# cp2k/dbcsr

Hardware: AMD Instinct MI355X
Metric: block-sparse multiply GFLOP/s (fp64) (higher is better)
Workload: dtype f64; 1 GPU; config2_32768_23x23_fill10_fp64; M=32768, c_nblks=2030625, nproducts=29207882, k_passes=1, parallelism=1 GPU

## Files before the change

### dbcsr_amd/csrc/mm_aux.h

```cpp
#ifndef DBCSR_AMD_MM_AUX_H
#define DBCSR_AMD_MM_AUX_H
#include "mm_epilogue.h"

namespace dbcsr_amd {

template <typename T>
__global__ void __launch_bounds__(256) checksum_blocks(const int* __restrict__ row_p, const int* __restrict__ col_i,
                                                       const int64_t* __restrict__ blk_p, const T* __restrict__ data,
                                                       const int* __restrict__ rs, const int* __restrict__ cs,
                                                       const int64_t* __restrict__ roff, const int64_t* __restrict__ coff, int nbr,
                                                       double* __restrict__ row_sums) {
  const int lane = threadIdx.x & 63;
  const int row = (blockIdx.x * blockDim.x + threadIdx.x) >> 6;
  if (row >= nbr) return;
  const int m = rs[row];
  double s2 = 0.0, sp = 0.0;
  for (int b = row_p[row]; b < row_p[row + 1]; ++b) {
    const int c = col_i[b];
    const int n = cs[c];
    const T* d = data + blk_p[b];
    for (int e = lane; e < m * n; e += 64) {
      const double x = (double)d[e];
      const int r = e % m, cc = e / m;
      s2 += x * x;
      sp += x * log(fabs((double)(roff[row] + r + 1) * (double)(coff[c] + cc + 1)));
    }
  }
  s2 = wave_sum(s2);
  sp = wave_sum(sp);
  if (lane == 0) {
    row_sums[2 * row] = s2;
    row_sums[2 * row + 1] = sp;
  }
}

__global__ void __launch_bounds__(256) checksum_final(const double* __restrict__ row_sums, int nbr, double* __restrict__ out2) {
  __shared__ double r2[256], rp[256];
  double s2 = 0.0, sp = 0.0;
  for (int i = threadIdx.x; i < nbr; i += 256) {
    s2 += row_sums[2 * i];
    sp += row_sums[2 * i + 1];
  }
  r2[threadIdx.x] = s2;
  rp[threadIdx.x] = sp;
  __syncthreads();
  for (int off = 128; off > 0; off >>= 1) {
    if ((int)threadIdx.x < off) {
      r2[threadIdx.x] += r2[threadIdx.x + off];
      rp[threadIdx.x] += rp[threadIdx.x + off];
    }
    __syncthreads();
  }
  if (threadIdx.x == 0) {
    out2[0] = r2[0];
    out2[1] = rp[0];
  }
}

__device__ __forceinline__ uint64_t larnv_block_seed(int irow, int nrow, int icol, int ival) {
  long long ivm = ((long long)ival) % 65536;
  if (ivm < 0) ivm += 65536;
  long long map = (((long long)irow - 1 + (long long)icol * (long long)nrow) * (1 + ivm)) * 2 + 1;
  const uint64_t s4 = (uint64_t)(map % 4096);
  map /= 4096;
  const uint64_t s3 = (uint64_t)((map ^ 3541) % 4096);
  map /= 4096;
  const uint64_t s2 = (uint64_t)((map ^ 1153) % 4096);
  map /= 4096;
  const uint64_t s1 = (uint64_t)((map ^ 2029) % 4096);
  return (s1 << 36) | (s2 << 24) | (s3 << 12) | s4;
}

__device__ __forceinline__ uint64_t pow48(uint64_t base, uint64_t e) {
  const uint64_t mask = (1ull << 48) - 1;
  uint64_t r = 1;
  base &= mask;
  while (e) {
    if (e & 1) r = (r * base) & mask;
    base = (base * base) & mask;
    e >>= 1;
  }
  return r;
}

__global__ void __launch_bounds__(256) fill_random_f64(const int* __restrict__ row_p, const int* __restrict__ col_i,
// ... 322 lines not shown
struct Window {
  int r0, r1, c0, c1;
};

__global__ void __launch_bounds__(256) crop_flags(const int* __restrict__ row_p, const int* __restrict__ col_i, const int* __restrict__ rs,
                                                  const int* __restrict__ cs, const int64_t* __restrict__ roff,
                                                  const int64_t* __restrict__ coff, int nbr, Window w, int* __restrict__ keep,
                                                  int* __restrict__ blk_nze, int* __restrict__ row_keep) {
  const int lane = threadIdx.x & 63;
  const int row = (blockIdx.x * blockDim.x + threadIdx.x) >> 6;
  if (row >= nbr) return;
  const int m = rs[row];
  const bool row_in = roff[row] + m - 1 >= w.r0 && roff[row] <= w.r1;
  int cnt = 0;
  for (int b = row_p[row] + lane; b < row_p[row + 1]; b += 64) {
    const int c = col_i[b], n = cs[c];
    const int k = (row_in && coff[c] + n - 1 >= w.c0 && coff[c] <= w.c1) ? 1 : 0;
    keep[b] = k;
    blk_nze[b] = k ? m * n : 0;
    cnt += k;
  }
  cnt = wave_sum(cnt);
  if (lane == 0) row_keep[row] = cnt;
}

template <typename T>
__global__ void __launch_bounds__(256) crop_compact(const int* __restrict__ row_p, const int* __restrict__ col_i,
                                                    const int64_t* __restrict__ blk_p, const T* __restrict__ data,
                                                    const int* __restrict__ rs, const int* __restrict__ cs,
                                                    const int64_t* __restrict__ roff, const int64_t* __restrict__ coff, int nbr, Window w,
                                                    const int* __restrict__ keep, const int64_t* __restrict__ newidx,
                                                    const int64_t* __restrict__ newoff, int* __restrict__ d_col_i,
                                                    int64_t* __restrict__ d_blk_p, T* __restrict__ d_data) {
  const int lane = threadIdx.x & 63;
  const int row = (blockIdx.x * blockDim.x + threadIdx.x) >> 6;
  if (row >= nbr) return;
  const int m = rs[row];
  const int64_t r_base = roff[row];
  for (int b = row_p[row]; b < row_p[row + 1]; ++b) {
    if (!keep[b]) continue;
    const int64_t t = newidx[b], off = newoff[b];
    const int c = col_i[b];
    if (lane == 0) {
      d_col_i[t] = c;
      d_blk_p[t] = off;
    }
    const int ne = m * cs[c];
    const int64_t c_base = coff[c];
    const T* src = data + blk_p[b];
    T* dst = d_data + off;
    for (int e = lane; e < ne; e += 64) {
      const int64_t gr = r_base + e % m, gc = c_base + e / m;
      dst[e] = (gr >= w.r0 && gr <= w.r1 && gc >= w.c0 && gc <= w.c1) ? src[e] : T(0);
    }
  }
}

template <typename T>
__global__ void __launch_bounds__(256) scale_window(const int* __restrict__ row_p, const int* __restrict__ col_i,
                                                    const int64_t* __restrict__ blk_p, T* __restrict__ data, const int* __restrict__ rs,
                                                    const int* __restrict__ cs, const int64_t* __restrict__ roff,
                                                    const int64_t* __restrict__ coff, int nbr, Window w, T beta) {
  const int lane = threadIdx.x & 63;
  const int row = (blockIdx.x * blockDim.x + threadIdx.x) >> 6;
  if (row >= nbr) return;
  const int m = rs[row];
  const int64_t r_base = roff[row];
  if (r_base + m - 1 < w.r0 || r_base > w.r1) return;
  for (int b = row_p[row]; b < row_p[row + 1]; ++b) {
    const int c = col_i[b], n = cs[c];
    const int64_t c_base = coff[c];
    if (c_base + n - 1 < w.c0 || c_base > w.c1) continue;
    T* blk = data + blk_p[b];
    for (int e = lane; e < m * n; e += 64) {
      const int64_t gr = r_base + e % m, gc = c_base + e / m;
      if (gr >= w.r0 && gr <= w.r1 && gc >= w.c0 && gc <= w.c1) blk[e] *= beta;
    }
  }
}



constexpr int kStatSlots = 8192;
__global__ void __launch_bounds__(256) build_work(const int* __restrict__ order, int64_t npos, const Desc* __restrict__ descs, int64_t nblk,
                                                  const Entry* __restrict__ entries, Work* __restrict__ work) {
  const int64_t pos = (int64_t)blockIdx.x * blockDim.x + threadIdx.x;
  if (pos >= npos) return;
  const int cb = order[pos];
  Work w;
  w.c_off = 0, w.cin_off = -1, w.prod_start = 0, w.prod_cnt = -1, w.m = 0, w.n = 0, w.a_lo = 0, w.b_lo = 0, w.w = 0, w.cb = cb;
  if (cb >= 0 && cb < nblk) {
    const Desc d = descs[cb];
    w.c_off = d.c_off, w.cin_off = d.cin_off, w.prod_start = d.prod_start, w.prod_cnt = d.prod_cnt, w.m = d.m, w.n = d.n;
    if (d.prod_cnt > 0) {
      const Entry e = entries[d.prod_start];
      w.a_lo = e.a_lo, w.b_lo = e.b_lo, w.w = e.w;
    }
  }
  work[pos] = w;
}

__global__ void __launch_bounds__(256) mnk_histogram(const Desc* __restrict__ descs, int64_t nblk, const Entry* __restrict__ entries,
                                                     unsigned long long* __restrict__ keys, unsigned long long* __restrict__ counts,
                                                     int* __restrict__ overflow) {
  const int64_t cb = (int64_t)blockIdx.x * blockDim.x + threadIdx.x;
  if (cb >= nblk) return;
  const Desc d = descs[cb];
  const Entry* e = entries + d.prod_start;
  unsigned long long run_key = 0, run_cnt = 0;
  auto flush = [&]() {
    if (!run_cnt) return;
    unsigned h = (unsigned)((run_key * 0x9E3779B97F4A7C15ull) >> 40) & (kStatSlots - 1);
    for (int probe = 0; probe < kStatSlots; ++probe) {
      const unsigned long long prev = atomicCAS(&keys[h], 0ull, run_key);
      if (prev == 0ull || prev == run_key) {
        atomicAdd(&counts[h], run_cnt);
        return;
      }
      h = (h + 1) & (kStatSlots - 1);
    }
    *overflow = 1;
  };
  for (int p = 0; p < d.prod_cnt; ++p) {
    const unsigned long long key = (unsigned long long)(uint16_t)d.m | ((unsigned long long)(uint16_t)d.n << 16) |
                                   ((unsigned long long)(unsigned)e[p].ks() << 32) | (1ull << 63);
    if (key != run_key) {
      flush();
      run_key = key;
      run_cnt = 0;
    }
    ++run_cnt;
  }
  flush();
}

}
#endif
```

### dbcsr_amd/csrc/mm_choose.h

```cpp
#ifndef DBCSR_AMD_MM_CHOOSE_H
#define DBCSR_AMD_MM_CHOOSE_H

#include <algorithm>
#include <cstddef>
#include <cstdint>
#include <cstdio>

namespace dbcsr_amd {

#define DBCSR_AMD_HOT_SIZES(X) \
  X(9) X(10) X(11) X(12) X(13) X(14) X(15) X(16) X(17) X(18) X(19) X(20) X(21) X(22) X(23) X(24) X(25) X(26) X(27) X(28) X(29) X(30) X(31) X(32)
#define DBCSR_AMD_DMA_SIZES(X) X(13) X(16) X(23) X(32)
#define DBCSR_AMD_F32_DIRECT_SIZES(X) X(16) X(24) X(32)
#define DBCSR_AMD_MID_SHAPES(X)                                                                             \
  X(6, 8) X(6, 9) X(6, 10) X(6, 11) X(6, 12)                                                                \
  X(7, 9) X(7, 10) X(7, 11) X(7, 12)                                                                        \
  X(8, 6) X(8, 8) X(8, 9) X(8, 10) X(8, 11) X(8, 12)                                                        \
  X(9, 6) X(9, 7) X(9, 8) X(9, 9) X(9, 10) X(9, 11) X(9, 12)                                                \
  X(10, 6) X(10, 7) X(10, 8) X(10, 9) X(10, 10) X(10, 11) X(10, 12)                                         \
  X(11, 6) X(11, 7) X(11, 8) X(11, 9) X(11, 10) X(11, 11) X(11, 12)                                         \
  X(12, 6) X(12, 7) X(12, 8) X(12, 9) X(12, 10) X(12, 11) X(12, 12)

#define DBCSR_AMD_IS_(S_) || s == S_
static inline bool hot_f64_has(int m, int n, int k) { const int s = m; return m == n && m == k && (false DBCSR_AMD_HOT_SIZES(DBCSR_AMD_IS_)); }
static inline bool dma_f64_has(int stages, int m, int n, int k) { const int s = m; return stages >= 2 && stages <= 4 && m == n && m == k && (false DBCSR_AMD_DMA_SIZES(DBCSR_AMD_IS_)); }
static inline bool f32_direct_has(int m, int n, int k) { const int s = m; return m == n && m == k && (false DBCSR_AMD_F32_DIRECT_SIZES(DBCSR_AMD_IS_)); }
#undef DBCSR_AMD_IS_
static inline bool big_f64_has(int tm, int tn) { return tm >= 2 && tm <= 5 && tn >= 2 && tn <= 5; }
static inline int big_tiles(int size) { return std::max(2, ((size + 7) / 8 + 1) / 2); }
static inline bool z64_has(int ma, int nc) { return ma >= 1 && ma <= 4 && nc >= 1 && nc <= 4; }
static inline int z64_tiles(int size) { return std::max(1, (std::min(size, 32) + 7) / 8); }
static inline constexpr int z64_slice_bytes(int ma, int nc) { return 8 * (8 * ma + 1) * 16 + 8 * nc * 9 * 16; }
static inline bool mid_f64_has(int rb, int cb) {
#define DBCSR_AMD_IS_(A_, B_) || (rb == A_ && cb == B_)
  return false DBCSR_AMD_MID_SHAPES(DBCSR_AMD_IS_);
#undef DBCSR_AMD_IS_
}

static inline bool mid_f64_serves(int m, int n, int class_mode) {
  const int rb = (m + 3) / 4, cb = (n + 3) / 4;
  const int lo = rb < cb ? rb : cb, hi = rb < cb ? cb : rb;
  if (lo < 6 || hi > 12 || hi < 8) return false;
  if (hi >= 11) return lo <= 10 || (m % 4 == 0 && n % 4 == 0);
  if (hi >= 9) return true;
  return class_mode > 0 && (lo == 8 || (lo == 6 && class_mode != 3));
}

struct SizeFacts {
  int max_m = 0, max_k = 0, max_n = 0, min_m = 0, min_k = 0, min_n = 0;
  int hot_m = 0, hot_n = 0, hot_k = 0;
  int hot_cnt_m = 0, hot_cnt_k = 0, hot_cnt_n = 0;
  int units_m = 0, units_cnt_m = 0, units_n = 0, units_cnt_n = 0;
  int nbr = 0, nbc = 0;
  int64_t c_nblks = 0, nproducts = 0, order_len = 0;
  bool cls_mode = false;
  int cls_m[3] = {0, 0, 0}, cls_n[3] = {0, 0, 0}, cls_k[3] = {0, 0, 0};
  bool retain = false;
  int canonical_c = 0;
  bool filter_active = false;
  bool fp64 = true;
  int skip_empty = 0;
  bool cplx = false;

  bool sizes_within(int s) const { return max_m <= s && max_k <= s && max_n <= s && min_m >= 1 && min_k >= 1 && min_n >= 1; }
  bool no_empty_dim() const { return min_m >= 1 && min_n >= 1 && min_k >= 1; }
  bool dominant_cube() const { return hot_m > 0 && hot_m == hot_n && hot_m == hot_k; }
  bool other_sizes() const { return hot_cnt_m < nbr || hot_cnt_n < nbc; }
};

struct Switches {
  int use_lds = 1;
  int use_pipe = -1, pipe_g = 8;
  int use_hot = 1;
  int use_tiny = 1;
  int use_small = 2;
  int small_group = 0;
  int use_mid = 1;
  int use_big = 1;
  int use_work = 1;
  int use_classes = 1;
  int wg_waves = 0;
  int f32_direct = 1;
};

struct LabSwitches {
#ifdef DBCSR_AMD_EXPERIMENTS
#define DBCSR_AMD_LAB_INT_ int
#else
#define DBCSR_AMD_LAB_INT_ static constexpr int
#endif
  DBCSR_AMD_LAB_INT_ dbg = 0;
  DBCSR_AMD_LAB_INT_ dma_stages = 0;
  DBCSR_AMD_LAB_INT_ hot_persistent = 0;
  DBCSR_AMD_LAB_INT_ hot_variant = 0;
  DBCSR_AMD_LAB_INT_ lds_pad = 0;
  DBCSR_AMD_LAB_INT_ class_g = 1;
  DBCSR_AMD_LAB_INT_ class_streams = 1;
  DBCSR_AMD_LAB_INT_ row_group = 0;
  DBCSR_AMD_LAB_INT_ f32_group = 0;
  DBCSR_AMD_LAB_INT_ f64_group = 0;
  DBCSR_AMD_LAB_INT_ use_tile = 0;
  DBCSR_AMD_LAB_INT_ use_band = 0;
#undef DBCSR_AMD_LAB_INT_
  bool variant_active() const { return (dbg & ~32) != 0 || dma_stages != 0 || hot_persistent != 0 || hot_variant != 0; }
};

static inline void top3_sizes(const int* hist, int* out) {
  int used[3] = {-1, -1, -1};
  for (int r = 0; r < 3; ++r) {
    int best = 0, bc = 0;
    for (int sz = 1; sz <= 32; ++sz)
      if (hist[sz] > bc && sz != used[0] && sz != used[1]) best = sz, bc = hist[sz];
    out[r] = best;
    used[r] = best ? best : -1;
  }
}
static inline void choose_classes(SizeFacts* f, const Switches& sw, const int* hist) {
  f->cls_mode = false;
  const bool hot_cube = f->hot_m >= 9 && f->dominant_cube();
  if (sw.use_classes > 0 && f->sizes_within(32) && !(f->max_m <= 4 && f->max_n <= 4) && (sw.use_classes > 1 || (!hot_cube && f->c_nblks >= 200000))) {
    top3_sizes(hist, f->cls_m);
    top3_sizes(hist + 33, f->cls_n);
    top3_sizes(hist + 66, f->cls_k);
    f->cls_mode = f->cls_m[0] > 0 && f->cls_n[0] > 0 && f->cls_k[0] > 0;
  }
}

enum class Family {
  f64_tiny, f64_small8, f64_mid, f64_classes, f64_hot, f64_pipe, f64_lds, f64_big, f64_generic, f32_classes, f32_direct, f32_hot, f32_lds, f32_generic,
  f64_group, f64_tile, f64_band, f64_dma, f64_persistent, f32_group,
  z64
};

struct NumericChoice {
  Family family = Family::f64_generic;
  char name[96] = "";
  int ww = 4;
  bool work = false, norms = false, leaves_norms = false;
  unsigned grid = 0;
  size_t lds_bytes = 0;
  int flags = 0;
  int lds_a = 0, lds_wave = 0, maxt = 0;
  int mid_rb = 0, mid_cb = 0, mid_class_mode = 0;
  int depth = 0, group = 0;
  bool slim = false;
  int variant = 0, group_R = 0;
};

static inline int choose_wg_waves(const SizeFacts& f, const Switches& sw) { return sw.wg_waves > 0 ? sw.wg_waves : (f.nproducts <= 32 * f.c_nblks ? 1 : 4); }

static inline void choose_mid_shape(const SizeFacts& f, const Switches& sw, const LabSwitches& lab, int* mid_rb, int* mid_cb) {
  *mid_rb = *mid_cb = 0;
  if (!(f.fp64 && sw.use_big && sw.use_mid && sw.use_lds && !f.cls_mode && f.max_m <= 48 && f.max_n <= 48 && f.no_empty_dim() && f.order_len > 0 &&
        !lab.variant_active() && sw.use_hot && sw.use_pipe != 1))
    return;
  const bool dom = f.hot_m > 0 && f.hot_n > 0, all_in = (f.min_m > 24 && f.min_n > 24) || f.max_m > 32 || f.max_n > 32;
  const int dm = dom ? f.hot_m : (all_in ? f.max_m : 0), dn = dom ? f.hot_n : (all_in ? f.max_n : 0);
  if (dm > 0 && dn > 0 && mid_f64_serves(dm, dn, 0)) *mid_rb = (dm + 3) / 4, *mid_cb = (dn + 3) / 4;
  if (*mid_rb && !dom) {
    const int mu = (std::max(f.max_m, f.max_n) + 3) / 4, fb = (mu > 10 || *mid_rb > 10 || *mid_cb > 10) ? 12 : 10;
    const bool single = *mid_rb == fb && *mid_cb == fb;
    const bool most = 10ll * f.units_cnt_m >= 8ll * f.nbr && 10ll * f.units_cnt_n >= 8ll * f.nbc && mid_f64_serves(4 * f.units_m, 4 * f.units_n, 0);
// ... 146 lines not shown
```

### dbcsr_amd/csrc/mm_engine.hip

```cpp
#include <hip/hip_runtime.h>

#include <cstdio>
#include <cstdlib>
#include <cstring>
#include <algorithm>
#include <new>
#include <vector>

#include "../../include/dbcsr_amd_mm.h"
#include "common.h"
#include "smm_core.h"
#include "mm_types.h"
#include "mm_complex.h"
#include "mm_jit.h"

#include "mm_workspace.h"
#include "mm_symbolic.h"
#include "mm_numeric_f64.h"
#include "mm_numeric_f64_big.h"
#include "mm_numeric_f64_small.h"
#include "mm_mid.h"
#include "mm_numeric_f32.h"
#include "mm_numeric_z64.h"
#include "mm_aux.h"
#include "mm_algebra.h"
#include "mm_elementwise.h"
#include "mm_blocklist.h"
#include "mm_multivec.h"
#include "mm_rank_update.h"
#include "mm_block_inverse.h"
#include "mm_block_scale.h"
#include "mm_dense.h"
#include "mm_submatrix.h"
#include "mm_csr.h"
#ifdef DBCSR_AMD_EXPERIMENTS
#include "mm_lab_api.h"
#include "mm_group.h"
#include "mm_group64.h"
#include "mm_dma.h"
#include "mm_tile_index.h"
#include "mm_band_index.h"
#endif
namespace dbcsr_amd {

#include "mm_engine_state.h"
#include "mm_engine_env.h"
#include "mm_engine_launch.h"
#include "mm_engine_plan.h"
#ifdef DBCSR_AMD_EXPERIMENTS
#include "mm_engine_lab.h"
#endif


static int build_product_lists(Engine* E, bool reuse, const dbcsr_amd_bcsr* a, const dbcsr_amd_bcsr* b, const dbcsr_amd_bcsr* c_in, dbcsr_amd_bcsr* c_out,
                               hipStream_t st) {
  const int nbr = E->facts.nbr, W = E->W, nbc = b->nblkcols, nJ = (nbc + 63) / 64;
  const int64_t nblk = E->facts.c_nblks;
  const uint32_t* cin_bm = E->have_cin ? E->cin_bm.p : nullptr;
  const int* cin_pre = E->have_cin ? E->cin_pre.p : nullptr;
  if (reuse) {
    ACC_CHECK(hipMemcpyAsync(c_out->col_i, E->plan_c_col_i.p, sizeof(int32_t) * (size_t)nblk, hipMemcpyDeviceToDevice, st));
    ACC_CHECK(hipMemcpyAsync(c_out->blk_p, E->plan_c_blk_p.p, sizeof(int64_t) * (size_t)nblk, hipMemcpyDeviceToDevice, st));
  } else if (E->rows_kernels) {
    if (E->tmp_i32.ensure((size_t)nblk + 1)) return -1;
    ACC_CHECK(hipMemsetAsync(E->tmp_i32.p, 0, sizeof(int) * (size_t)nblk, st));
    hipLaunchKernelGGL(fill_products_rows, grid_for((int64_t)nbr * 64), dim3(256), 0, st, a->row_p, a->col_i, a->blk_p, a->col_blk_size, b->row_p,
                       b->col_i, b->blk_p, E->c_bm.p, E->c_pre.p, c_out->row_p, E->prod_start.p, nbr, W, E->tmp_i32.p, E->entries.p, E->filter);
    hipLaunchKernelGGL(finish_descs_grid, grid_for((int64_t)nbr * nJ * 64), dim3(256), 0, st, c_in->row_p, c_in->blk_p, c_out->row_blk_size,
                       c_out->col_blk_size, cin_bm, cin_pre, E->c_bm.p, E->c_pre.p, c_out->row_p, E->c_blk_p_ws.p, E->prod_start.p,
                       E->prod_cnt.p, nbr, W, nJ, c_out->col_i, c_out->blk_p, E->descs.p);
  } else if (E->grid_kernels) {
    hipLaunchKernelGGL(fill_products_grid, grid_for((int64_t)nbr * nJ * 64), dim3(256), 0, st, a->row_p, a->col_i, a->blk_p, b->row_p,
                       b->blk_p, c_in->row_p, c_in->blk_p, a->row_blk_size, a->col_blk_size, b->col_blk_size, E->b_bm.p, E->b_pre.p,
                       cin_bm, cin_pre, E->c_bm.p, E->c_pre.p, c_out->row_p, E->prod_start.p, E->c_blk_p_ws.p, nbr, nbc, W, nJ, c_out->col_i,
                       c_out->blk_p, E->descs.p, E->entries.p, E->filter);
  } else {
    hipLaunchKernelGGL(fill_products, grid_for((int64_t)nbr * W), dim3(256), 0, st, a->row_p, a->col_i, a->blk_p, b->row_p, b->blk_p,
                       c_in->row_p, c_in->blk_p, a->row_blk_size, a->col_blk_size, b->col_blk_size, E->b_bm.p, E->b_pre.p,
                       cin_bm, cin_pre, E->c_bm.p, E->c_pre.p, c_out->row_p, E->prod_start.p, E->c_blk_p_ws.p, nbr, W, c_out->col_i, c_out->blk_p,
                       E->descs.p, E->entries.p);
  }
  return 0;
}

template <typename T>
static NumericArgs<T> numeric_args(Engine* E, hipStream_t st, const dbcsr_amd_bcsr* a, const dbcsr_amd_bcsr* b, const dbcsr_amd_bcsr* c_in,
                                   const dbcsr_amd_bcsr* c_out, T alpha, T beta, const Work* work, double* norms, bool reuse) {
  return NumericArgs<T>{st, E->descs.p, E->facts.c_nblks, E->entries.p, static_cast<const T*>(a->data), static_cast<const T*>(b->data),
                        static_cast<T*>(c_out->data), static_cast<const T*>(c_in->data), alpha, beta, E->facts.skip_empty, E->order.p, work, norms,
                        a, b, c_out, reuse};
}

static int launch_classes_f64(Engine* E, const NumericArgs<double>& p, const NumericChoice& c) {
  const SizeFacts& F = E->facts;
  int njit = 0, ngen = 0, nmid = 0, jit_mask = 0, nlaunch = 0;
  const int nside = E->lab.class_streams > 1 ? E->lab.class_streams - 1 : 0;
  if (nside) {
    if (!E->fork_ev) ACC_CHECK(hipEventCreateWithFlags(&E->fork_ev, hipEventDisableTiming));
    ACC_CHECK(hipEventRecord(E->fork_ev, p.st));
    for (int i = 0; i < nside; ++i) {
      if (!E->side_stream[i]) {
        ACC_CHECK(hipStreamCreateWithFlags(&E->side_stream[i], hipStreamNonBlocking));
        ACC_CHECK(hipEventCreateWithFlags(&E->join_ev[i], hipEventDisableTiming));
      }
      ACC_CHECK(hipStreamWaitEvent(E->side_stream[i], E->fork_ev, 0));
    }
  }
  for (int k = 0; k < kNumClasses; ++k) {
    if (E->cls_len[k] == 0) continue;
    NumericArgs<double> q = p.segment(E->cls_off[k]);
    const int slot = nlaunch++ % (nside + 1);
    if (slot) q.st = E->side_stream[slot - 1];
    const unsigned npos = (unsigned)(8 * E->cls_len[k]);
    const int cm = k < 9 ? F.cls_m[k / 3] : 0, cn = k < 9 ? F.cls_n[k % 3] : 0;
    ClassKernel ck;
    if (k < 9 && c.mid_class_mode && mid_f64_serves(cm, cn, c.mid_class_mode)) {
      if (!launch_mid_f64(q, (cm + 3) / 4, (cn + 3) / 4, false, npos, (std::max(cm, cn) + 3) / 4)) return -1;
      ++nmid;
      jit_mask |= 1 << k;
    } else if (k < 9 && cm > 0 && cn > 0 && jit_class_kernel(cm, cn, F.cls_k[0], F.cls_k[1], F.cls_k[2], E->lab.class_g, &ck) == 0) {
      long nblk_l = (long)q.nblk;
      void* args[] = {&q.descs, &nblk_l, &q.entries, &q.a, &q.b, &q.c_out, &q.c_in, &q.alpha, &q.beta, &q.skip_empty, &q.order, &q.work, &q.norms};
      const unsigned cw = E->lab.class_g == 1 ? (unsigned)c.ww : 4u;
      ACC_CHECK(hipModuleLaunchKernel(ck.fn, npos / cw / (unsigned)E->lab.class_g, 1, 1, 64 * cw, 1, 1, (unsigned)(cw * ck.wave_lds), q.st, args, nullptr));
      ++njit;
      jit_mask |= 1 << k;
    } else {
      launch_lds_f64(q, c, (unsigned)(8 * E->cls_len[k] / 4) * 4u / (unsigned)c.ww);
      ++ngen;
    }
  }
  for (int i = 0; i < nside; ++i) {
    ACC_CHECK(hipEventRecord(E->join_ev[i], E->side_stream[i]));
    ACC_CHECK(hipStreamWaitEvent(p.st, E->join_ev[i], 0));
  }
  if (p.norms) {
    ClassSet cs;
    for (int r = 0; r < 3; ++r) cs.m[r] = F.cls_m[r], cs.n[r] = F.cls_n[r];
    cs.jit_mask = jit_mask;
    hipLaunchKernelGGL(block_norms_unserved_classes, grid_for(p.nblk * 64), dim3(256), 0, p.st, p.descs, p.nblk, p.c_out, cs, p.norms);
  }
  char slab[24] = "";
  if (nmid > 0) snprintf(slab, sizeof slab, "%d slab + ", nmid);
  snprintf(E->last_kernel, sizeof E->last_kernel, "%s%d jit + %s%d generic launches; m {%d,%d,%d} n {%d,%d,%d} k {%d,%d,%d}]", c.name, njit, slab, ngen,
           F.cls_m[0], F.cls_m[1], F.cls_m[2], F.cls_n[0], F.cls_n[1], F.cls_n[2], F.cls_k[0], F.cls_k[1], F.cls_k[2]);
  return 0;
}

static int launch_f64(Engine* E, const NumericChoice& c, const NumericArgs<double>& p, const LabSwitches& lab) {
  const SizeFacts& F = E->facts;
  const int64_t npos = 8 * F.order_len;
  snprintf(E->last_kernel, sizeof E->last_kernel, "%s", c.name);
  if (p.norms && c.leaves_norms) E->norms_data = p.c_out, E->norms_nblks = p.nblk;
  switch (c.family) {
    case Family::f64_tiny:
      if (c.grid > 0) launch_tiny_f64(p, c, F.max_k <= 4);
      return 0;
    case Family::f64_small8:
      if (c.grid > 0) launch_small_f64(p, c, npos);
      return 0;
    case Family::f64_mid:
      return launch_mid_f64(p, c.mid_rb, c.mid_cb, F.min_m != F.max_m || F.min_n != F.max_n, c.grid, (std::max(F.max_m, F.max_n) + 3) / 4) ? 0 : -1;
    case Family::f64_classes: return launch_classes_f64(E, p, c);
    case Family::f64_hot: return launch_hot_f64(p, c, F.hot_m, F.hot_n, F.hot_k, c.flags, c.variant) ? 0 : -1;
    case Family::f64_pipe: launch_pipe_f64(p, c, npos); return 0;
    case Family::f64_lds: launch_lds_f64(p, c, c.grid); return 0;
    case Family::f64_big: return launch_big_f64(p, c, big_tiles(F.max_m), big_tiles(F.max_n)) ? 0 : -1;
    case Family::f64_generic:
      hipLaunchKernelGGL(mm_numeric_f64, dim3(c.grid), dim3(256), 0, p.st, p.descs, p.nblk, p.entries, p.a, p.b, p.c_out, p.c_in, p.alpha, p.beta, c.flags);
      return 0;
#ifdef DBCSR_AMD_EXPERIMENTS
    case Family::f64_group: case Family::f64_tile: case Family::f64_band: case Family::f64_dma: case Family::f64_persistent: return launch_lab_f64(E, c, p, lab);
#endif
    default: return -1;
  }
}

static int launch_f32(Engine* E, const NumericChoice& c, const NumericArgs<float>& p) {
  const SizeFacts& F = E->facts;
  snprintf(E->last_kernel, sizeof E->last_kernel, "%s", c.name);
  switch (c.family) {
    case Family::f32_classes:
      for (int k = 0; k < kNumClasses; ++k)
        if (E->cls_len[k] != 0) launch_lds_f32(p.segment(E->cls_off[k]), c, (unsigned)(8 * E->cls_len[k] / c.ww));
      return 0;
    case Family::f32_direct: return launch_hot_f32_direct(p, c, F.hot_m, F.hot_n, F.hot_k, c.flags, c.slim) ? 0 : -1;
    case Family::f32_hot: return launch_hot_f32(p, c, F.hot_m, F.hot_n, F.hot_k) ? 0 : -1;
    case Family::f32_lds: launch_lds_f32(p, c, c.grid); return 0;
    case Family::f32_generic:
      hipLaunchKernelGGL(mm_numeric_f32, dim3(c.grid), dim3(256), 0, p.st, p.descs, p.nblk, p.entries, p.a, p.b, p.c_out, p.c_in, p.alpha, p.beta, c.flags);
      return 0;
#ifdef DBCSR_AMD_EXPERIMENTS
    case Family::f32_group: {
      const int rc = run_group_f32(E, p, c.group_R);
      if (rc == 0 && F.other_sizes()) launch_hot_f32_direct(p, c, F.hot_m, F.hot_n, F.hot_k, c.flags | 2, false);
      if (rc != 1) return rc;
      LabSwitches lab = E->lab;
      lab.f32_group = 0;
      return launch_f32(E, choose_numeric(F, E->sw, lab), p);
    }
#endif
    default: return -1;
  }
}

static int launch_z64_family(Engine* E, const NumericChoice& c, const NumericArgs<z64>& p) {
  const SizeFacts& F = E->facts;
  snprintf(E->last_kernel, sizeof E->last_kernel, "%s", c.name);
  if (c.family != Family::z64) return -1;
  return launch_z64(p, c, z64_tiles(F.max_m), z64_tiles(F.max_n), 8 * F.order_len) ? 0 : -1;
}

static int numeric_phase(void* handle, libsmm_acc_data_t datatype, const double alpha[2], const dbcsr_amd_bcsr* a, const dbcsr_amd_bcsr* b,
                         const double beta[2], const dbcsr_amd_bcsr* c_in, dbcsr_amd_bcsr* c_out, void* stream);

}

using namespace dbcsr_amd;

extern "C" {

int dbcsr_amd_mm_create(void** handle) {
  if (!handle) return -1;
  Engine* E = new (std::nothrow) Engine();
  if (!E) return -1;
  hipError_t e = hipHostMalloc(reinterpret_cast<void**>(&E->host_scalars), 16 * sizeof(int64_t), hipHostMallocDefault);
  if (e != hipSuccess) {
    delete E;
    return check(e, "hipHostMalloc", __FILE__, __LINE__);
  }
  if (hipHostMalloc(reinterpret_cast<void**>(&E->cls_host_hist), 3 * 33 * sizeof(int), hipHostMallocDefault) != hipSuccess ||
      hipHostMalloc(reinterpret_cast<void**>(&E->cls_host_lens), (2 * kNumClasses + 1) * sizeof(int64_t), hipHostMallocDefault) != hipSuccess)
    return -1;
  if (hipHostMalloc(reinterpret_cast<void**>(&E->plan_host_flag), sizeof(int), hipHostMallocDefault) != hipSuccess) return -1;
  engine_read_env(E);
  for (int i = 0; i < 3; ++i) {
    e = hipEventCreate(&E->ev[i]);
    if (e != hipSuccess) return check(e, "hipEventCreate", __FILE__, __LINE__);
  }
  *handle = E;
  return 0;
}

int dbcsr_amd_mm_timing(void* handle, float* ms_fill, float* ms_numeric) {
  Engine* E = static_cast<Engine*>(handle);
  if (!E || !E->timed) return -1;
  ACC_CHECK(hipEventSynchronize(E->ev[2]));
  float f = 0.f, n = 0.f;
  ACC_CHECK(hipEventElapsedTime(&f, E->ev[0], E->ev[1]));
  ACC_CHECK(hipEventElapsedTime(&n, E->ev[1], E->ev[2]));
  if (ms_fill) *ms_fill = f;
  if (ms_numeric) *ms_numeric = n;
  return 0;
}

int dbcsr_amd_mm_destroy(void* handle) {
  if (!handle) return 0;
  Engine* E = static_cast<Engine*>(handle);
  if (E->host_scalars) (void)hipHostFree(E->host_scalars);
  if (E->plan_host_flag) (void)hipHostFree(E->plan_host_flag);
  if (E->cls_host_hist) (void)hipHostFree(E->cls_host_hist);
  if (E->cls_host_lens) (void)hipHostFree(E->cls_host_lens);
  for (int i = 0; i < 3; ++i)
    if (E->ev[i]) (void)hipEventDestroy(E->ev[i]);
  for (int i = 0; i < 3; ++i) {
    if (E->side_stream[i]) (void)hipStreamDestroy(E->side_stream[i]);
    if (E->join_ev[i]) (void)hipEventDestroy(E->join_ev[i]);
  }
  if (E->fork_ev) (void)hipEventDestroy(E->fork_ev);
  delete E;
  return 0;
}

int dbcsr_amd_mm_symbolic(void* handle, const dbcsr_amd_bcsr* a, const dbcsr_amd_bcsr* b, const dbcsr_amd_bcsr* c_in,
                          int retain_sparsity, int32_t* c_out_row_p, dbcsr_amd_mm_counts* counts, void* stream) {
  return dbcsr_amd_mm_symbolic_filtered(handle, dbcsr_type_real_8, 1.0, 0.0, a, b, c_in, retain_sparsity, c_out_row_p, counts, stream);
}

int dbcsr_amd_mm_symbolic_filtered(void* handle, libsmm_acc_data_t datatype, double alpha, double filter_eps, const dbcsr_amd_bcsr* a,
                                   const dbcsr_amd_bcsr* b, const dbcsr_amd_bcsr* c_in, int retain_sparsity, int32_t* c_out_row_p,
                                   dbcsr_amd_mm_counts* counts, void* stream) {
  Engine* E = static_cast<Engine*>(handle);
  if (!E || !a || !b || !c_in || !c_out_row_p || !counts) return -1;
  E->drop_pending = 0.0;
  engine_takes_work_areas(E);
  const bool filtering = filter_eps > 0.0;
  if (filtering && datatype != dbcsr_type_real_8 && datatype != dbcsr_type_real_4 && datatype != dbcsr_type_complex_8) return -10;
  if (a->nblkcols != b->nblkrows || a->nblkrows != c_in->nblkrows || b->nblkcols != c_in->nblkcols) {
    fprintf(stderr, "dbcsr_amd_mm_symbolic: incompatible block dimensions\n");
    return -2;
  }
  hipStream_t st = stream_of(stream);
  const int nbr = a->nblkrows, nbk = a->nblkcols, nbc = b->nblkcols;
  const int W = (nbc + 31) / 32;
  if (!filtering) {
    const int hit = plan_matches(E, a, b, c_in, retain_sparsity ? 1 : 0, st);
    if (hit < 0) return -1;
    if (hit) {
      long long off = 0;
      const void* ptr[12];
      long long n[12];
      plan_segments(a, b, c_in, ptr, n);
      for (int i = 0; i < 12; ++i) off += n[i];
      ACC_CHECK(hipMemcpyAsync(c_out_row_p, E->plan_words.p + off, sizeof(int32_t) * ((size_t)nbr + 1), hipMemcpyDeviceToDevice, st));
      *counts = E->plan_counts;
      E->norms_data = nullptr;
      E->filter = FilterArgs{nullptr, nullptr, 0.0f};
      E->valid = true;
      E->plan_hit = true;
      ++E->plan_hits;
      return 0;
    }
  }
  plan_invalidate(E);
  E->valid = false;
  E->facts.nbr = nbr;
  E->facts.nbc = nbc;
  E->W = W;
  E->facts.retain = retain_sparsity != 0;
  E->norms_data = nullptr;
  E->have_cin = c_in->nblks > 0;
  if (E->b_bm.ensure((size_t)nbk * W + 1) || E->b_pre.ensure((size_t)nbk * W + 1) || E->c_bm.ensure((size_t)nbr * W + 1) ||
      E->c_pre.ensure((size_t)nbr * W + 1) || E->row_nnz.ensure((size_t)nbr + 1) || E->dev_scalars.ensure(16))
    return -1;
  if (E->have_cin && (E->cin_bm.ensure((size_t)nbr * W + 1) || E->cin_pre.ensure((size_t)nbr * W + 1))) return -1;
  ACC_CHECK(hipMemsetAsync(E->dev_scalars.p, 0, 16 * sizeof(unsigned long long), st));
  {
    static const int init[6] = {0, -0x7fffffff, 0, -0x7fffffff, 0, -0x7fffffff};
    ACC_CHECK(hipMemcpyAsync(E->dev_scalars.p + 4, init, sizeof(init), hipMemcpyHostToDevice, st));
  }
  if (nbr == 0 || nbc == 0) {
    ACC_CHECK(hipMemsetAsync(c_out_row_p, 0, sizeof(int32_t) * ((size_t)nbr + 1), st));
    ACC_CHECK(hipStreamSynchronize(st));
    counts->c_nblks = counts->c_nze = counts->nproducts = counts->flop = 0;
    E->facts.c_nblks = 0;
    E->facts.nproducts = 0;
    E->grid_kernels = E->rows_kernels = false;
    E->facts.cls_mode = false;
    E->sym_bitmap = -1;
    E->sym_NP = E->sym_PW = E->sym_rowp_chunks = 0;
    E->valid = true;
    return 0;
  }
  ACC_CHECK(hipMemsetAsync(E->b_bm.p, 0, sizeof(uint32_t) * (size_t)nbk * W, st));
  if (nbk > 0) {
    hipLaunchKernelGGL(bitmap_from_index, grid_for((int64_t)nbk * 64), dim3(256), 0, st, b->row_p, b->col_i, nbk, W, E->b_bm.p);
    hipLaunchKernelGGL(row_prefix, grid_for((int64_t)nbk * 64), dim3(256), 0, st, E->b_bm.p, nbk, W, E->b_pre.p, (int*)nullptr);
  }
  if (E->have_cin) {
    ACC_CHECK(hipMemsetAsync(E->cin_bm.p, 0, sizeof(uint32_t) * (size_t)nbr * W, st));
    hipLaunchKernelGGL(bitmap_from_index, grid_for((int64_t)nbr * 64), dim3(256), 0, st, c_in->row_p, c_in->col_i, nbr, W,
                       E->cin_bm.p);
    hipLaunchKernelGGL(row_prefix, grid_for((int64_t)nbr * 64), dim3(256), 0, st, E->cin_bm.p, nbr, W, E->cin_pre.p, (int*)nullptr);
  }
  E->filter = FilterArgs{nullptr, nullptr, 0.0f};
  if (filtering) {
    if (E->a_norms.ensure((size_t)a->nblks + 1) || E->b_norms.ensure((size_t)b->nblks + 1)) return -1;
    const int sa = row_split(nbr, a->nblks), sb = row_split(nbk, b->nblks);
    if (datatype == dbcsr_type_real_8) {
      hipLaunchKernelGGL((bcsr_block_norms<double>), grid_for((int64_t)nbr * sa * 64), dim3(256), 0, st, a->row_p, a->col_i, a->blk_p,
                         static_cast<const double*>(a->data), a->row_blk_size, a->col_blk_size, nbr, sa, 1.0, E->a_norms.p, (double*)nullptr);
      hipLaunchKernelGGL((bcsr_block_norms<double>), grid_for((int64_t)nbk * sb * 64), dim3(256), 0, st, b->row_p, b->col_i, b->blk_p,
                         static_cast<const double*>(b->data), b->row_blk_size, b->col_blk_size, nbk, sb, alpha, E->b_norms.p, (double*)nullptr);
    } else if (datatype == dbcsr_type_complex_8) {
      hipLaunchKernelGGL((bcsr_block_norms<z64>), grid_for((int64_t)nbr * sa * 64), dim3(256), 0, st, a->row_p, a->col_i, a->blk_p,
                         static_cast<const z64*>(a->data), a->row_blk_size, a->col_blk_size, nbr, sa, 1.0, E->a_norms.p, (double*)nullptr);
      hipLaunchKernelGGL((bcsr_block_norms<z64>), grid_for((int64_t)nbk * sb * 64), dim3(256), 0, st, b->row_p, b->col_i, b->blk_p,
                         static_cast<const z64*>(b->data), b->row_blk_size, b->col_blk_size, nbk, sb, alpha, E->b_norms.p, (double*)nullptr);
    } else {
      hipLaunchKernelGGL((bcsr_block_norms<float>), grid_for((int64_t)nbr * sa * 64), dim3(256), 0, st, a->row_p, a->col_i, a->blk_p,
                         static_cast<const float*>(a->data), a->row_blk_size, a->col_blk_size, nbr, sa, 1.0, E->a_norms.p, (double*)nullptr);
      hipLaunchKernelGGL((bcsr_block_norms<float>), grid_for((int64_t)nbk * sb * 64), dim3(256), 0, st, b->row_p, b->col_i, b->blk_p,
                         static_cast<const float*>(b->data), b->row_blk_size, b->col_blk_size, nbk, sb, alpha, E->b_norms.p, (double*)nullptr);
    }
    E->filter = FilterArgs{E->a_norms.p, E->b_norms.p, (float)filter_eps};
  }
  SymbolicSizes sizes;
  sizes.nbr = nbr, sizes.nbk = nbk, sizes.nbc = nbc, sizes.a_nblks = a->nblks, sizes.b_nblks = b->nblks;
  sizes.filtering = filtering, sizes.retain = retain_sparsity != 0, sizes.forced = E->force_symbolic;
  SymbolicChoice sym = choose_symbolic_pattern(sizes);
  if (sym.bitmap_rows) {
    if (E->have_cin)
      ACC_CHECK(hipMemcpyAsync(E->c_bm.p, E->cin_bm.p, sizeof(uint32_t) * (size_t)nbr * W, hipMemcpyDeviceToDevice, st));
    else
      ACC_CHECK(hipMemsetAsync(E->c_bm.p, 0, sizeof(uint32_t) * (size_t)nbr * W, st));
    hipLaunchKernelGGL(c_bitmap_rows_filtered, grid_for((int64_t)nbr * 64), dim3(256), 0, st, a->row_p, a->col_i, b->row_p, b->col_i, nbr, W,
                       E->facts.canonical_c, E->filter, E->c_bm.p);
  } else if (filtering)
    hipLaunchKernelGGL(c_bitmap_filtered, grid_for((int64_t)nbr * ((nbc + 63) / 64) * 64), dim3(256), 0, st, a->row_p, a->col_i, b->row_p,
                       E->b_bm.p, E->b_pre.p, E->have_cin ? E->cin_bm.p : (const uint32_t*)nullptr, nbr, nbc, W, (nbc + 63) / 64,
                       retain_sparsity ? 1 : 0, E->facts.canonical_c, E->filter, E->c_bm.p);
  else
    hipLaunchKernelGGL(c_bitmap, grid_for((int64_t)nbr * W), dim3(256), 0, st, a->row_p, a->col_i, E->b_bm.p,
                       E->have_cin ? E->cin_bm.p : (const uint32_t*)nullptr, nbr, W, retain_sparsity ? 1 : 0, E->facts.canonical_c, E->c_bm.p);
  hipLaunchKernelGGL(row_prefix, grid_for((int64_t)nbr * 64), dim3(256), 0, st, E->c_bm.p, nbr, W, E->c_pre.p, E->row_nnz.p);
  int64_t* dsc = reinterpret_cast<int64_t*>(E->dev_scalars.p);
  if (exclusive_scan<int32_t>(E, E->row_nnz.p, nbr, c_out_row_p, dsc + 0, true, st)) return -1;
  if (E->sw.use_classes > 0 && E->cls_hist.ensure(3 * 33)) return -1;
  hipLaunchKernelGGL(block_size_stats, dim3(3), dim3(256), 0, st, a->row_blk_size, nbr, a->col_blk_size, nbk, b->col_blk_size, nbc,
                     reinterpret_cast<int*>(E->dev_scalars.p + 4), reinterpret_cast<int*>(E->dev_scalars.p + 8), reinterpret_cast<int*>(E->dev_scalars.p + 11),
                     E->sw.use_classes > 0 ? E->cls_hist.p : (int*)nullptr);
  if (E->sw.use_classes > 0) ACC_CHECK(hipMemcpyAsync(E->cls_host_hist, E->cls_hist.p, 3 * 33 * sizeof(int), hipMemcpyDeviceToHost, st));
  ACC_CHECK(hipMemcpyAsync(E->host_scalars, dsc, 13 * sizeof(int64_t), hipMemcpyDeviceToHost, st));
  ACC_CHECK(hipStreamSynchronize(st));
  const int64_t c_nblks = E->host_scalars[0];
  {
    const int* mx = reinterpret_cast<const int*>(E->host_scalars + 4);
    E->facts.max_m = mx[0]; E->facts.min_m = -mx[1];
    E->facts.max_k = mx[2]; E->facts.min_k = -mx[3];
    E->facts.max_n = mx[4]; E->facts.min_n = -mx[5];
    if (E->facts.max_k > 0xffff || E->facts.max_m > 0x7fff || E->facts.max_n > 0x7fff) {
      fprintf(stderr, "dbcsr_amd_mm_symbolic: block sizes above 32767 (m, n) / 65535 (k) are not supported (packed 16-bit extents)\n");
      return -1;
    }
    const int* md = reinterpret_cast<const int*>(E->host_scalars + 8);
    const bool dominant = 10ll * md[1] >= 9ll * nbr && 10ll * md[3] >= 9ll * nbk && 10ll * md[5] >= 9ll * nbc;
    E->facts.hot_m = dominant ? md[0] : 0;
    E->facts.hot_k = dominant ? md[2] : 0;
    E->facts.hot_n = dominant ? md[4] : 0;
    E->facts.hot_cnt_m = md[1], E->facts.hot_cnt_k = md[3], E->facts.hot_cnt_n = md[5];
    const int* um = reinterpret_cast<const int*>(E->host_scalars + 11);
    E->facts.units_m = um[0], E->facts.units_cnt_m = um[1], E->facts.units_n = um[2], E->facts.units_cnt_n = um[3];
  }
  E->facts.c_nblks = c_nblks;
  choose_classes(&E->facts, E->sw, E->cls_host_hist);
  double mean_k = E->facts.max_k, mean_n = E->facts.max_n;
  if (E->sw.use_classes > 0 && E->facts.max_k <= 32 && E->facts.max_n <= 32 && E->facts.min_k >= 1 && E->facts.min_n >= 1) {
    double sk = 0, ck = 0, sn = 0, cn = 0;
    for (int sz = 1; sz <= 32; ++sz) {
      sn += (double)sz * E->cls_host_hist[33 + sz];
      cn += E->cls_host_hist[33 + sz];
      sk += (double)sz * E->cls_host_hist[66 + sz];
      ck += E->cls_host_hist[66 + sz];
    }
    if (ck > 0 && cn > 0) mean_k = sk / ck, mean_n = sn / cn;
  }
  const int64_t b_bytes_est = (int64_t)((double)b->nblks * mean_k * mean_n * (double)sizeof(double));
  int NP = 1, PW = W;
  choose_panels(W, b_bytes_est, E->panel_bytes, &NP, &PW);
  const int R = (nbr + 7) / 8;
  int RG = E->lab.row_group > 0 ? E->lab.row_group : 1;
  RG = std::max(1, std::min(RG, R));
  const int NG = (R + RG - 1) / RG;
  const int nkeys = (E->facts.cls_mode ? kNumClasses : 1) * 8 * NP * (E->facts.cls_mode ? R : NG);
  if (E->order_cnt.ensure((size_t)nkeys + 1) || E->order_base.ensure((size_t)nkeys + 1)) return -1;
  if (E->facts.cls_mode) {
    if (E->cls_row.ensure((size_t)nbr + 1) || E->cls_col.ensure((size_t)nbc + 1) || E->cls_col_bm.ensure((size_t)4 * W + 1) ||
        E->cls_lens.ensure(2 * kNumClasses + 1) || E->cls_vpos.ensure((size_t)nbr + 1) || E->cls_vrow.ensure((size_t)nbr + 1))
      return -1;
    hipLaunchKernelGGL(class_ids, grid_for(nbr), dim3(256), 0, st, a->row_blk_size, nbr, E->facts.cls_m[0], E->facts.cls_m[1], E->facts.cls_m[2], E->cls_row.p);
    hipLaunchKernelGGL(class_ids, grid_for(nbc), dim3(256), 0, st, b->col_blk_size, nbc, E->facts.cls_n[0], E->facts.cls_n[1], E->facts.cls_n[2], E->cls_col.p);
    hipLaunchKernelGGL(class_col_bitmaps, grid_for(W), dim3(256), 0, st, E->cls_col.p, nbc, W, E->cls_col_bm.p);
    hipLaunchKernelGGL(class_row_deal, dim3(1), dim3(256), 0, st, E->cls_row.p, nbr, E->cls_vpos.p, E->cls_vrow.p);
    hipLaunchKernelGGL(order_count_cls, grid_for(nkeys), dim3(256), 0, st, E->c_bm.p, E->cls_row.p, E->cls_col_bm.p, E->cls_vrow.p, nbr, W, PW, NP, R,
                       E->order_cnt.p);
    if (exclusive_scan<int64_t>(E, E->order_cnt.p, nkeys, E->order_base.p, nullptr, false, st)) return -1;
    hipLaunchKernelGGL(order_len_cls, dim3(1), dim3(1), 0, st, E->order_base.p, c_nblks, NP, R, E->cls_lens.p);
    ACC_CHECK(hipMemcpyAsync(E->cls_host_lens, E->cls_lens.p, (2 * kNumClasses + 1) * sizeof(int64_t), hipMemcpyDeviceToHost, st));
  } else {
  hipLaunchKernelGGL(order_count, grid_for(nkeys), dim3(256), 0, st, E->c_pre.p, E->row_nnz.p, nbr, W, PW, NP, NG, RG, E->order_cnt.p);
  if (exclusive_scan<int64_t>(E, E->order_cnt.p, nkeys, E->order_base.p, nullptr, false, st)) return -1;
  hipLaunchKernelGGL(order_len, dim3(1), dim3(1), 0, st, E->order_base.p, c_nblks, NP, NG, dsc + 7);
  }
  if (E->prod_cnt.ensure((size_t)c_nblks + 1) || E->blk_nze.ensure((size_t)c_nblks + 1) || E->prod_start.ensure((size_t)c_nblks + 1) ||
      E->c_blk_p_ws.ensure((size_t)c_nblks + 1))
    return -1;
  const int nJ = (nbc + 63) / 64;
  sym = choose_symbolic_count(sizes, sym, c_nblks);
  E->grid_kernels = sym.grid_kernels;
  E->rows_kernels = sym.rows_kernels;
  E->sym_bitmap = sym.bitmap_rows ? 2 : (filtering ? 1 : 0);
  E->sym_NP = NP, E->sym_PW = PW;
  E->sym_rowp_chunks = (int)(((int64_t)nbr + kScanChunk - 1) / kScanChunk);
  if (E->rows_kernels) {
    ACC_CHECK(hipMemsetAsync(E->prod_cnt.p, 0, sizeof(int) * (size_t)c_nblks, st));
    hipLaunchKernelGGL(block_sizes_rows, grid_for((int64_t)nbr * W), dim3(256), 0, st, E->c_bm.p, E->c_pre.p, c_out_row_p, a->row_blk_size,
                       b->col_blk_size, nbr, W, E->blk_nze.p);
    hipLaunchKernelGGL(count_products_rows, grid_for((int64_t)nbr * 64), dim3(256), 0, st, a->row_p, a->col_i, a->row_blk_size, a->col_blk_size,
                       b->col_blk_size, b->row_p, b->col_i, E->c_bm.p, E->c_pre.p, c_out_row_p, nbr, W, E->prod_cnt.p, E->dev_scalars.p + 3,
                       E->filter);
  } else if (E->grid_kernels)
    hipLaunchKernelGGL(count_products_grid, grid_for((int64_t)nbr * nJ * 64), dim3(256), 0, st, a->row_p, a->col_i, a->row_blk_size,
                       a->col_blk_size, b->col_blk_size, E->b_bm.p, E->c_bm.p, E->c_pre.p, c_out_row_p, nbr, nbc, W, nJ,
                       E->prod_cnt.p, E->blk_nze.p, E->dev_scalars.p + 3, b->row_p, E->b_pre.p, E->filter);
  else
    hipLaunchKernelGGL(count_products, grid_for((int64_t)nbr * W), dim3(256), 0, st, a->row_p, a->col_i, a->row_blk_size,
                       a->col_blk_size, b->col_blk_size, E->b_bm.p, E->c_bm.p, E->c_pre.p, c_out_row_p, nbr, W, E->prod_cnt.p,
                       E->blk_nze.p, E->dev_scalars.p + 3);
  if (exclusive_scan<int64_t>(E, E->prod_cnt.p, c_nblks, E->prod_start.p, dsc + 2, false, st)) return -1;
  if (exclusive_scan<int64_t>(E, E->blk_nze.p, c_nblks, E->c_blk_p_ws.p, dsc + 1, false, st)) return -1;
  ACC_CHECK(hipMemcpyAsync(E->host_scalars, dsc, 8 * sizeof(int64_t), hipMemcpyDeviceToHost, st));
  ACC_CHECK(hipStreamSynchronize(st));
  E->facts.order_len = E->host_scalars[7];
  if (E->facts.cls_mode) {
    for (int c = 0; c < kNumClasses; ++c) {
      E->cls_len[c] = E->cls_host_lens[c];
      E->cls_off[c] = E->cls_host_lens[kNumClasses + c];
    }
    const int64_t total = E->cls_host_lens[2 * kNumClasses];
    E->facts.order_len = total / 8;
    if (E->order.ensure((size_t)total + 64)) return -1;
    if (total > 0) {
      ACC_CHECK(hipMemsetAsync(E->order.p, 0xff, sizeof(int) * ((size_t)total + 64), st));
      hipLaunchKernelGGL(order_fill_cls, grid_for((int64_t)nbr * W), dim3(256), 0, st, E->c_bm.p, E->c_pre.p, c_out_row_p, E->cls_row.p,
                         E->cls_col_bm.p, E->order_base.p, E->cls_lens.p, E->cls_vpos.p, nbr, W, PW, NP, R, E->order.p);
    }
  } else {
  if (E->order.ensure((size_t)(8 * E->facts.order_len) + 64)) return -1;
  if (E->facts.order_len > 0) {
    ACC_CHECK(hipMemsetAsync(E->order.p, 0xff, sizeof(int) * ((size_t)(8 * E->facts.order_len) + 64), st));
    hipLaunchKernelGGL(order_fill, grid_for((int64_t)nbr * W), dim3(256), 0, st, E->c_bm.p, E->c_pre.p, E->row_nnz.p, c_out_row_p,
                       E->order_base.p, nbr, W, PW, NP, NG, RG, E->facts.order_len, E->order.p);
  }
  }
  counts->c_nblks = E->host_scalars[0];
  counts->c_nze = E->host_scalars[1];
  counts->nproducts = E->host_scalars[2];
  counts->flop = E->host_scalars[3];
  E->facts.c_nblks = counts->c_nblks;
  E->facts.nproducts = counts->nproducts;
  E->valid = true;
  ++E->plan_misses;
  if (!filtering) {
    if (plan_save(E, a, b, c_in, retain_sparsity ? 1 : 0, c_out_row_p, *counts, st)) return -1;
  } else {
    plan_invalidate(E);
  }
  return check(hipGetLastError(), "dbcsr_amd_mm_symbolic", __FILE__, __LINE__);
}

int dbcsr_amd_mm_numeric(void* handle, libsmm_acc_data_t datatype, double alpha, const dbcsr_amd_bcsr* a, const dbcsr_amd_bcsr* b,
                         double beta, const dbcsr_amd_bcsr* c_in, dbcsr_amd_bcsr* c_out, void* stream) {
  const double al[2] = {alpha, 0.0}, be[2] = {beta, 0.0};
  return numeric_phase(handle, datatype, al, a, b, be, c_in, c_out, stream);
}

int dbcsr_amd_mm_numeric_z(void* handle, const double alpha[2], const dbcsr_amd_bcsr* a, const dbcsr_amd_bcsr* b, const double beta[2],
                           const dbcsr_amd_bcsr* c_in, dbcsr_amd_bcsr* c_out, void* stream) {
  if (!alpha || !beta) return -1;
  return numeric_phase(handle, dbcsr_type_complex_8, alpha, a, b, beta, c_in, c_out, stream);
}

#include "mm_engine_ops.h"
#include "mm_engine_algebra.h"
#include "mm_engine_elementwise.h"
#include "mm_engine_blocklist.h"
#include "mm_engine_csr.h"

}

namespace dbcsr_amd {

static int numeric_phase(void* handle, libsmm_acc_data_t datatype, const double alpha_z[2], const dbcsr_amd_bcsr* a, const dbcsr_amd_bcsr* b,
                         const double beta_z[2], const dbcsr_amd_bcsr* c_in, dbcsr_amd_bcsr* c_out, void* stream) {
  const double alpha = alpha_z[0], beta = beta_z[0];
  Engine* E = static_cast<Engine*>(handle);
  if (!E || !E->valid || !a || !b || !c_in || !c_out) {
    fprintf(stderr, "dbcsr_amd_mm_numeric: no valid symbolic phase for this handle\n");
    return -1;
  }
  if (datatype != dbcsr_type_real_8 && datatype != dbcsr_type_real_4 && datatype != dbcsr_type_complex_8) return -10;
  hipStream_t st = stream_of(stream);
  SizeFacts& F = E->facts;
  const int64_t nblk = F.c_nblks;
  if (nblk == 0) return 0;
  const bool reuse = E->plan_hit && E->plan_numeric;
  if (!reuse) {
    E->work_built = false;
#ifdef DBCSR_AMD_EXPERIMENTS
    E->ls.forget_plan();
#endif
  }
  if (E->entries.ensure((size_t)F.nproducts + 1) || E->descs.ensure((size_t)nblk + 1)) return -1;
  ACC_CHECK(hipEventRecord(E->ev[0], st));
  if (int rc = build_product_lists(E, reuse, a, b, c_in, c_out, st)) return rc;
  F.nbc = b->nblkcols;
  F.fp64 = datatype == dbcsr_type_real_8;
  F.cplx = datatype == dbcsr_type_complex_8;
  F.filter_active = E->filter.a_norms != nullptr;
  F.skip_empty = (c_out->data == c_in->data && F.retain && beta == 1.0 && beta_z[1] == 0.0) ? 1 : 0;
  const NumericChoice ch = choose_numeric(F, E->sw, E->lab);
  const Work* work = nullptr;
  if (ch.work) {
    const int64_t npos = 8 * F.order_len;
    if (!(reuse && E->work_built)) {
      if (E->work.ensure((size_t)npos + 1)) return -1;
      hipLaunchKernelGGL(build_work, grid_for(npos), dim3(256), 0, st, E->order.p, npos, E->descs.p, nblk, E->entries.p, E->work.p);
      E->work_built = true;
    }
    work = E->work.p;
  }
  double* norms = nullptr;
  E->norms_data = nullptr;
  if (ch.norms) {
    if (E->norms64.ensure((size_t)nblk + 1)) return -1;
    norms = E->norms64.p;
  }
  const double drop = norms ? E->drop_pending : 0.0;
  E->drop_pending = 0.0;
  E->unwritten_below = 0.0;
  if (norms) {
    hipLaunchKernelGGL(store_scalar_f64, dim3(1), dim3(1), 0, st, norms + nblk, drop);
    E->unwritten_below = drop;
  }
  ACC_CHECK(hipEventRecord(E->ev[1], st));
  if ((F.cplx ? launch_z64_family(E, ch, numeric_args<z64>(E, st, a, b, c_in, c_out, z64(alpha, alpha_z[1]), z64(beta, beta_z[1]), work, norms, reuse))
       : F.fp64 ? launch_f64(E, ch, numeric_args<double>(E, st, a, b, c_in, c_out, alpha, beta, work, norms, reuse), E->lab)
                : launch_f32(E, ch, numeric_args<float>(E, st, a, b, c_in, c_out, (float)alpha, (float)beta, work, norms, reuse))) != 0) {
    fprintf(stderr, "dbcsr_amd_mm_numeric: launching %s failed\n", E->last_kernel);
    return -1;
  }
  ACC_CHECK(hipEventRecord(E->ev[2], st));
  E->timed = true;
  c_out->nblks = nblk;
  if (E->plan_saved && !E->plan_numeric) {
    if (E->plan_c_col_i.ensure((size_t)nblk + 1) || E->plan_c_blk_p.ensure((size_t)nblk + 1)) return -1;
    ACC_CHECK(hipMemcpyAsync(E->plan_c_col_i.p, c_out->col_i, sizeof(int32_t) * (size_t)nblk, hipMemcpyDeviceToDevice, st));
    ACC_CHECK(hipMemcpyAsync(E->plan_c_blk_p.p, c_out->blk_p, sizeof(int64_t) * (size_t)nblk, hipMemcpyDeviceToDevice, st));
    E->plan_numeric = true;
  }
  return check(hipGetLastError(), "dbcsr_amd_mm_numeric", __FILE__, __LINE__);
}

}
```

### dbcsr_amd/csrc/mm_engine_env.h

```cpp
#ifndef DBCSR_AMD_MM_ENGINE_ENV_H
#define DBCSR_AMD_MM_ENGINE_ENV_H

static void engine_read_env(Engine* E) {
  if (const char* k = getenv("DBCSR_AMD_MM_KERNEL")) {
    E->sw.use_lds = strcmp(k, "direct") != 0;
    E->sw.use_pipe = strcmp(k, "pipe") == 0 ? 1 : (strcmp(k, "lds1") == 0 ? 0 : -1);
#ifdef DBCSR_AMD_EXPERIMENTS
    if (strncmp(k, "dma", 3) == 0 && k[3] >= '2' && k[3] <= '4') E->lab.dma_stages = k[3] - '0';
#endif
  }
  if (const char* k = getenv("DBCSR_AMD_MM_PIPE_G")) E->sw.pipe_g = std::max(1, atoi(k));
  if (const char* k = getenv("DBCSR_AMD_MM_CLASSES")) E->sw.use_classes = atoi(k);
  if (const char* k = getenv("DBCSR_AMD_MM_WORK")) E->sw.use_work = atoi(k);
  if (const char* k = getenv("DBCSR_AMD_MM_WG_WAVES")) {
    const int w = atoi(k);
    if (w == 1 || w == 2 || w == 4) E->sw.wg_waves = w;
  }
  if (const char* k = getenv("DBCSR_AMD_MM_PLAN")) E->use_plan = atoi(k);
  if (const char* k = getenv("DBCSR_AMD_MM_HOT")) E->sw.use_hot = atoi(k);
  if (const char* k = getenv("DBCSR_AMD_MM_TINY")) E->sw.use_tiny = atoi(k);
  if (const char* k = getenv("DBCSR_AMD_MM_SMALL")) E->sw.use_small = atoi(k);
  if (const char* k = getenv("DBCSR_AMD_MM_SMALL_G")) E->sw.small_group = std::min(64, std::max(0, atoi(k)));
  if (const char* k = getenv("DBCSR_AMD_MM_F32_DIRECT")) E->sw.f32_direct = atoi(k);
  if (const char* k = getenv("DBCSR_AMD_MM_BIG")) E->sw.use_big = atoi(k);
  if (const char* k = getenv("DBCSR_AMD_MM_MID")) E->sw.use_mid = atoi(k);
  if (const char* k = getenv("DBCSR_AMD_MM_SYMBOLIC")) {
    E->force_symbolic = strcmp(k, "word") == 0 ? 1 : (strcmp(k, "grid") == 0 ? 2 : (strcmp(k, "rows") == 0 ? 3 : 0));
  }
  if (const char* k = getenv("DBCSR_AMD_MM_PANEL_MB")) E->panel_bytes = panel_bytes_of_mb(atoll(k));
#ifdef DBCSR_AMD_EXPERIMENTS
  if (const char* k = getenv("DBCSR_AMD_MM_F32_GROUP")) {
    const int r = atoi(k);
    E->lab.f32_group = (r >= 2 && r <= 4) ? r : (r < 0 ? -1 : 0);
  }
  if (const char* k = getenv("DBCSR_AMD_MM_F64_GROUP")) E->lab.f64_group = atoi(k);
  if (const char* k = getenv("DBCSR_AMD_MM_GROUP_PANEL_MB")) E->ls.group_panel_bytes = panel_bytes_of_mb(atoll(k));
  if (const char* k = getenv("DBCSR_AMD_MM_CLASS_G")) {
    const int g = atoi(k);
    E->lab.class_g = (g == 2 || g == 4 || g == 8) ? g : 1;
  }
  if (const char* k = getenv("DBCSR_AMD_MM_DBG")) E->lab.dbg = atoi(k);
  if (const char* k = getenv("DBCSR_AMD_ALG_COLSUMS")) E->ls.alg_col_variant = atoi(k);
  if (const char* k = getenv("DBCSR_AMD_MULTIVEC_WAVES")) E->ls.multivec_waves = atoi(k);
  {
    const char* k = getenv("DBCSR_AMD_MM_POISON");
    g_devbuf_poison = k ? (atoi(k) & 255) : -1;
  }
  if (const char* k = getenv("DBCSR_AMD_MM_HOT_VARIANT")) E->lab.hot_variant = atoi(k);
  if (const char* k = getenv("DBCSR_AMD_MM_HOT_PERSISTENT")) E->lab.hot_persistent = atoi(k);
  if (const char* k = getenv("DBCSR_AMD_MM_HOT_XCDS")) E->ls.hot_xcd_mask = (unsigned)strtoul(k, nullptr, 0) & 0xffu;
  if (const char* k = getenv("DBCSR_AMD_MM_TILE")) E->lab.use_tile = atoi(k);
  if (const char* k = getenv("DBCSR_AMD_MM_TILE_WINDOW")) E->ls.tile_window = atoi(k);
  if (const char* k = getenv("DBCSR_AMD_MM_TILE_RDV")) E->ls.tile_rdv = atoi(k);
  if (const char* k = getenv("DBCSR_AMD_MM_TILE_PUB")) E->ls.tile_pub = atoi(k);
  if (const char* k = getenv("DBCSR_AMD_MM_TILE_PREFETCH")) E->ls.tile_prefetch = atoi(k);
  if (const char* k = getenv("DBCSR_AMD_MM_TILE_KNOBS")) E->ls.tile_knobs = atoi(k);
  if (const char* k = getenv("DBCSR_AMD_MM_TILE_SHAPE")) E->ls.tile_shape = atoi(k) == 1 ? 1 : 0;
  if (const char* k = getenv("DBCSR_AMD_MM_BAND")) E->lab.use_band = atoi(k);
  if (const char* k = getenv("DBCSR_AMD_MM_BAND_DEPTH")) E->ls.band_depth = atoi(k);
  if (const char* k = getenv("DBCSR_AMD_MM_BAND_BPOL")) E->ls.band_bpol = atoi(k) == 1 ? 1 : 0;
  if (const char* k = getenv("DBCSR_AMD_MM_BAND_KNOBS")) E->ls.band_knobs = atoi(k);
  if (const char* k = getenv("DBCSR_AMD_MM_BAND_WINDOW")) E->ls.band_window = atoi(k);
  if (const char* k = getenv("DBCSR_AMD_MM_BAND_SHAPE")) E->ls.band_shape = atoi(k) == 0 ? 0 : 1;
  if (const char* k = getenv("DBCSR_AMD_MM_LDS_PAD")) E->lab.lds_pad = atoi(k);
  if (const char* k = getenv("DBCSR_AMD_MM_CLASS_STREAMS")) E->lab.class_streams = std::min(4, std::max(1, atoi(k)));
  if (const char* k = getenv("DBCSR_AMD_MM_ROW_GROUP")) E->lab.row_group = atoi(k);
#endif
}

#endif
```

### dbcsr_amd/csrc/mm_engine_launch.h

```cpp
#ifndef DBCSR_AMD_MM_ENGINE_LAUNCH_H
#define DBCSR_AMD_MM_ENGINE_LAUNCH_H


__global__ void __launch_bounds__(256) block_norms_other_sizes(const Desc* __restrict__ descs, int64_t nblk, const double* __restrict__ c_data,
                                                               int m, int n, double* __restrict__ norms) {
  const int lane = threadIdx.x & 63;
  const int64_t cb = ((int64_t)blockIdx.x * blockDim.x + threadIdx.x) >> 6;
  if (cb >= nblk) return;
  const Desc d = descs[cb];
  if (d.m == m && d.n == n) return;
  const double* x = c_data + d.c_off;
  double ss = 0.0;
  for (int e = lane; e < d.m * d.n; e += 64) ss += x[e] * x[e];
  ss = wave_sum(ss);
  if (lane == 0) norms[cb] = ss;
}

struct ClassSet {
  int m[3], n[3], jit_mask;
};
__global__ void __launch_bounds__(256) block_norms_unserved_classes(const Desc* __restrict__ descs, int64_t nblk, const double* __restrict__ c_data,
                                                                    ClassSet cs, double* __restrict__ norms) {
  const int lane = threadIdx.x & 63;
  const int64_t cb = ((int64_t)blockIdx.x * blockDim.x + threadIdx.x) >> 6;
  if (cb >= nblk) return;
  const Desc d = descs[cb];
  int rm = 3, rn = 3;
#pragma unroll
  for (int q = 2; q >= 0; --q) {
    if (cs.m[q] > 0 && d.m == cs.m[q]) rm = q;
    if (cs.n[q] > 0 && d.n == cs.n[q]) rn = q;
  }
  if (rm < 3 && rn < 3 && ((cs.jit_mask >> (3 * rm + rn)) & 1)) return;
  const double* x = c_data + d.c_off;
  double ss = 0.0;
  for (int e = lane; e < d.m * d.n; e += 64) ss += x[e] * x[e];
  ss = wave_sum(ss);
  if (lane == 0) norms[cb] = ss;
}


static bool launch_hot_f64(const NumericArgs<double>& p, const NumericChoice& c, int m, int n, int k, int flags, int variant) {
  if (!hot_f64_has(m, n, k)) return false;
  const dim3 grid(c.grid), block(64 * c.ww);
#ifdef DBCSR_AMD_EXPERIMENTS
  if (m == 23 && variant >= 1 && variant <= 6) {
    auto kern = variant == 1 ? mm_numeric_f64_hot<23, 23, 23, 1> : variant == 2 ? mm_numeric_f64_hot<23, 23, 23, 2> : variant == 3 ? mm_numeric_f64_hot<23, 23, 23, 3> :
                variant == 4 ? mm_numeric_f64_hot<23, 23, 23, 4> : variant == 5 ? mm_numeric_f64_hot<23, 23, 23, 5> : mm_numeric_f64_hot<23, 23, 23, 6>;
    hipLaunchKernelGGL(kern, grid, block, c.lds_bytes, p.st, p.descs, p.nblk, p.entries, p.a, p.b, p.c_out, p.c_in, p.alpha, p.beta, c.lds_a, c.lds_wave, flags,
                       p.order, p.work, p.norms);
    return true;
  }
#else
  (void)variant;
#endif
  switch (m) {
#define DBCSR_HOT_CASE(S_)                                                                                                                          \
  case S_:                                                                                                                                          \
    hipLaunchKernelGGL((mm_numeric_f64_hot<S_, S_, S_, 0>), grid, block, c.lds_bytes, p.st, p.descs, p.nblk, p.entries, p.a, p.b, p.c_out, p.c_in,  \
                       p.alpha, p.beta, c.lds_a, c.lds_wave, flags, p.order, p.work, p.norms);                                                     \
    return true;
    DBCSR_AMD_HOT_SIZES(DBCSR_HOT_CASE)
#undef DBCSR_HOT_CASE
    default: return false;
  }
}

#ifdef DBCSR_AMD_EXPERIMENTS
static bool launch_dma_f64(const NumericArgs<double>& p, const NumericChoice& c, int S, int m, int n, int k) {
  if (!dma_f64_has(S, m, n, k)) return false;
  switch (S * 64 + m) {
#define DBCSR_DMA_CASE(R_, S_)                                                                                                               \
  case R_ * 64 + S_:                                                                                                                          \
    hipLaunchKernelGGL((mm_numeric_f64_dma<S_, S_, S_, R_>), dim3(c.grid), dim3(64), (DmaRing<S_, S_, S_, R_>::BYTES), p.st, p.descs, p.nblk, \
                       p.entries, p.a, p.b, p.c_out, p.c_in, p.alpha, p.beta, c.flags, p.order);                                              \
    return true;
#define DBCSR_DMA_RINGS(S_) DBCSR_DMA_CASE(2, S_) DBCSR_DMA_CASE(3, S_) DBCSR_DMA_CASE(4, S_)
    DBCSR_AMD_DMA_SIZES(DBCSR_DMA_RINGS)
#undef DBCSR_DMA_RINGS
#undef DBCSR_DMA_CASE
    default: return false;
  }
}
#endif

static bool launch_hot_f32(const NumericArgs<float>& p, const NumericChoice& c, int m, int n, int k) {
  if (!hot_f64_has(m, n, k)) return false;
  switch (m) {
#define DBCSR_HOT_CASE(S_)                                                                                                                          \
  case S_:                                                                                                                                          \
    hipLaunchKernelGGL((mm_numeric_f32_hot<S_, S_, S_>), dim3(c.grid), dim3(64 * c.ww), f32_lds_bytes(c.ww), p.st, p.descs, p.nblk, p.entries, p.a, \
                       p.b, p.c_out, p.c_in, p.alpha, p.beta, c.flags, p.order);                                                                    \
    return true;
    DBCSR_AMD_HOT_SIZES(DBCSR_HOT_CASE)
#undef DBCSR_HOT_CASE
    default: return false;
  }
}

static bool launch_hot_f32_direct(const NumericArgs<float>& p, const NumericChoice& c, int m, int n, int k, int flags, bool slim) {
  if (!f32_direct_has(m, n, k)) return false;
  switch (m) {
#define DBCSR_DIRECT_CASE(S_)                                                                                                                      \
  case S_:                                                                                                                                         \
    hipLaunchKernelGGL((slim ? mm_numeric_f32_direct_slim<S_, S_, S_> : mm_numeric_f32_direct<S_, S_, S_>), dim3(c.grid), dim3(64 * c.ww),         \
                       slim ? (size_t)c.ww * f32d_wave_floats(S_) * sizeof(float) : f32_lds_bytes(c.ww), p.st, p.descs, p.nblk, p.entries, p.a, p.b, \
                       p.c_out, p.c_in, p.alpha, p.beta, flags, p.order);                                                                          \
    return true;
    DBCSR_AMD_F32_DIRECT_SIZES(DBCSR_DIRECT_CASE)
#undef DBCSR_DIRECT_CASE
    default: return false;
  }
}

static void launch_lds_f32(const NumericArgs<float>& p, const NumericChoice& c, unsigned grid) {
  hipLaunchKernelGGL(mm_numeric_f32_lds, dim3(grid), dim3(64 * c.ww), f32_lds_bytes(c.ww), p.st, p.descs, p.nblk, p.entries, p.a, p.b, p.c_out, p.c_in,
                     p.alpha, p.beta, c.flags, p.order);
}

static bool launch_big_f64(const NumericArgs<double>& p, const NumericChoice& c, int tm, int tn) {
  if (!big_f64_has(tm, tn) || c.grid == 0) return false;
  switch (tm * 8 + tn) {
#define DBCSR_BIG_CASE(A_, B_)                                                                                                                  \
  case A_ * 8 + B_:                                                                                                                             \
    hipLaunchKernelGGL((mm_numeric_f64_big<A_, B_>), dim3(c.grid), dim3(256), (size_t)big_lds_bytes(A_, B_), p.st, p.descs, p.nblk, p.entries,  \
                       p.a, p.b, p.c_out, p.c_in, p.alpha, p.beta, c.flags, p.order);                                                           \
    return true;
    DBCSR_BIG_CASE(2, 2) DBCSR_BIG_CASE(2, 3) DBCSR_BIG_CASE(2, 4) DBCSR_BIG_CASE(2, 5)
    DBCSR_BIG_CASE(3, 2) DBCSR_BIG_CASE(3, 3) DBCSR_BIG_CASE(3, 4) DBCSR_BIG_CASE(3, 5)
    DBCSR_BIG_CASE(4, 2) DBCSR_BIG_CASE(4, 3) DBCSR_BIG_CASE(4, 4) DBCSR_BIG_CASE(4, 5)
    DBCSR_BIG_CASE(5, 2) DBCSR_BIG_CASE(5, 3) DBCSR_BIG_CASE(5, 4) DBCSR_BIG_CASE(5, 5)
#undef DBCSR_BIG_CASE
    default: return false;
  }
}

static void launch_lds_f64(const NumericArgs<double>& p, const NumericChoice& c, unsigned grid) {
  auto kern = c.maxt == 1 ? mm_numeric_f64_lds<1> : c.maxt == 2 ? mm_numeric_f64_lds<2> : c.maxt == 3 ? mm_numeric_f64_lds<3> : mm_numeric_f64_lds<4>;
  hipLaunchKernelGGL(kern, dim3(grid), dim3(64 * c.ww), c.lds_bytes, p.st, p.descs, p.nblk, p.entries, p.a, p.b, p.c_out, p.c_in, p.alpha, p.beta, c.lds_a,
                     c.lds_wave, c.flags, p.order);
}

static void launch_pipe_f64(const NumericArgs<double>& p, const NumericChoice& c, int64_t npos) {
// ... 40 lines not shown
```

### dbcsr_amd/csrc/mm_engine_ops.h

```cpp
#ifndef DBCSR_AMD_MM_ENGINE_OPS_H
#define DBCSR_AMD_MM_ENGINE_OPS_H

static int init_c_any(void* handle, libsmm_acc_data_t datatype, double beta, double beta_im, const dbcsr_amd_bcsr* c_in, dbcsr_amd_bcsr* c_out,
                      void* stream) {
  Engine* E = static_cast<Engine*>(handle);
  if (E) E->plan_numeric = false;
  if (!E || !E->valid || !c_in || !c_out) {
    fprintf(stderr, "dbcsr_amd_mm_init_c: no valid symbolic phase for this handle\n");
    return -1;
  }
  if (datatype != dbcsr_type_real_8 && datatype != dbcsr_type_real_4 && datatype != dbcsr_type_complex_8) return -10;
  hipStream_t st = stream_of(stream);
  const int nbr = E->facts.nbr, W = E->W;
  const int64_t nblk = E->facts.c_nblks;
  engine_writes_values(E);
  c_out->nblks = nblk;
  if (nblk == 0) return 0;
  if (E->descs.ensure((size_t)nblk + 1)) return -1;
  hipLaunchKernelGGL(emit_index, grid_for((int64_t)nbr * W), dim3(256), 0, st, c_in->row_p, c_in->blk_p, c_out->row_blk_size,
                     c_out->col_blk_size, E->have_cin ? E->cin_bm.p : (const uint32_t*)nullptr,
                     E->have_cin ? E->cin_pre.p : (const int*)nullptr, E->c_bm.p, E->c_pre.p, c_out->row_p, E->c_blk_p_ws.p, nbr, W,
                     c_out->col_i, c_out->blk_p, E->descs.p);
  if (datatype == dbcsr_type_real_8)
    hipLaunchKernelGGL((init_c_blocks<double>), grid_for(nblk * 64), dim3(256), 0, st, E->descs.p, nblk,
// ... 413 lines not shown
  else if (datatype == dbcsr_type_real_4)
    hipLaunchKernelGGL((desym_fill<float>), grid_for((int64_t)nbr * 64), dim3(256), 0, st, src->row_p, src->col_i, src->blk_p,
                       static_cast<const float*>(src->data), src->row_blk_size, E->c_bm.p, E->c_pre.p, dst->row_p, E->c_blk_p_ws.p, nbr, W,
                       kind, mode, dst->col_i, dst->blk_p, static_cast<float*>(dst->data));
  else
    hipLaunchKernelGGL(twin_fill_z64, grid_for((int64_t)nbr * 64), dim3(256), 0, st, src->row_p, src->col_i, src->blk_p,
                       static_cast<const z64*>(src->data), src->row_blk_size, E->c_bm.p, E->c_pre.p, dst->row_p, E->c_blk_p_ws.p, nbr, W,
                       kind, mode, dst->col_i, dst->blk_p, static_cast<z64*>(dst->data));
  return check(hipGetLastError(), "dbcsr_amd_bcsr_twin_apply", __FILE__, __LINE__);
}

int dbcsr_amd_mm_stats(void* handle, dbcsr_amd_mnk_stat* out, int max_entries, int* n_entries, void* stream) {
  Engine* E = static_cast<Engine*>(handle);
  if (!E || !n_entries || (max_entries > 0 && !out)) return -1;
  *n_entries = 0;
  if (!E->valid || !E->timed || E->facts.c_nblks == 0) return 0;
  hipStream_t st = stream_of(stream);
  if (E->stat_table.ensure(2 * (size_t)kStatSlots + 2)) return -1;
  unsigned long long* keys = E->stat_table.p;
  unsigned long long* counts = keys + kStatSlots;
  int* overflow = reinterpret_cast<int*>(counts + kStatSlots);
  ACC_CHECK(hipMemsetAsync(keys, 0, sizeof(unsigned long long) * (2 * (size_t)kStatSlots + 2), st));
  hipLaunchKernelGGL(mnk_histogram, grid_for(E->facts.c_nblks), dim3(256), 0, st, E->descs.p, E->facts.c_nblks, E->entries.p, keys, counts, overflow);
  std::vector<unsigned long long> host(2 * (size_t)kStatSlots + 2);
  ACC_CHECK(hipMemcpyAsync(host.data(), keys, sizeof(unsigned long long) * host.size(), hipMemcpyDeviceToHost, st));
  ACC_CHECK(hipStreamSynchronize(st));
  if (*reinterpret_cast<const int*>(&host[2 * (size_t)kStatSlots])) {
    fprintf(stderr, "dbcsr_amd_mm_stats: more than %d distinct (m, n, k) triples\n", kStatSlots);
    return -1;
  }
  std::vector<dbcsr_amd_mnk_stat> all;
  for (int i = 0; i < kStatSlots; ++i)
    if (host[i]) {
      dbcsr_amd_mnk_stat r;
      r.m = (int32_t)(host[i] & 0xffffu);
      r.n = (int32_t)((host[i] >> 16) & 0xffffu);
      r.k = (int32_t)((host[i] >> 32) & 0x7fffffffu);
      r.reserved = 0;
      r.nproducts = (int64_t)host[kStatSlots + i];
      r.flop = 2ll * r.m * r.n * r.k * r.nproducts;
      all.push_back(r);
    }
  std::sort(all.begin(), all.end(), [](const dbcsr_amd_mnk_stat& a, const dbcsr_amd_mnk_stat& b) {
    return a.flop != b.flop ? a.flop > b.flop : (a.m != b.m ? a.m < b.m : (a.n != b.n ? a.n < b.n : a.k < b.k));
  });
  *n_entries = (int)all.size();
  for (int i = 0; i < (int)all.size() && i < max_entries; ++i) out[i] = all[i];
  return 0;
}

const char* dbcsr_amd_mm_kernel_name(libsmm_acc_data_t datatype) {
  return datatype == dbcsr_type_complex_8 ? "mm_numeric_z64" : datatype == dbcsr_type_real_4 ? "mm_numeric_f32" : "mm_numeric_f64";
}

const char* dbcsr_amd_mm_last_kernel(void* handle) {
  Engine* E = static_cast<Engine*>(handle);
  return E ? E->last_kernel : "";
}

const char* dbcsr_amd_mm_last_symbolic(void* handle) {
  Engine* E = static_cast<Engine*>(handle);
  if (!E) return "";
  static const char* const bitmap[] = {"none", "plain", "filtered", "rows_filtered"};
  snprintf(E->last_symbolic, sizeof E->last_symbolic, "bitmap=%s count=%s W=%d NP=%d PW=%d classes=%d rowp_chunks=%d plan=%s",
           bitmap[std::min(std::max(E->sym_bitmap, -1), 2) + 1], E->sym_bitmap < 0 ? "none" : (E->rows_kernels ? "rows" : (E->grid_kernels ? "grid" : "word")),
           E->W, E->sym_NP, E->sym_PW, E->facts.cls_mode ? 1 : 0, E->sym_rowp_chunks, E->plan_hit ? "hit" : "miss");
  return E->last_symbolic;
}

int dbcsr_amd_mm_expect_filter(void* handle, double eps) {
  Engine* E = static_cast<Engine*>(handle);
  if (!E || !(eps >= 0.0)) return -1;
  E->drop_pending = eps * eps;
  return 0;
}

int dbcsr_amd_mm_trust_plan(void* handle, int on) {
  Engine* E = static_cast<Engine*>(handle);
  if (!E) return -1;
  E->plan_trusted = on != 0;
  return 0;
}

int dbcsr_amd_mm_plan_stats(void* handle, int64_t* reused, int64_t* built) {
  Engine* E = static_cast<Engine*>(handle);
  if (!E) return -1;
  if (reused) *reused = E->plan_hits;
  if (built) *built = E->plan_misses;
  return 0;
}

#ifdef DBCSR_AMD_EXPERIMENTS
int dbcsr_amd_mm_tile_stats(void* handle, int* waves_gave_up, int* list_mismatches) {
  Engine* E = static_cast<Engine*>(handle);
  if (!E) return -1;
  if (strncmp(E->last_kernel, "mm_numeric_f64_tile", 19) != 0 || !E->ls.tile_flags.p) return 1;
  int h[4] = {0, 0, 0, 0};
  ACC_CHECK(hipDeviceSynchronize());
  ACC_CHECK(hipMemcpy(h, E->ls.tile_flags.p, sizeof h, hipMemcpyDeviceToHost));
  if (waves_gave_up) *waves_gave_up = h[0];
  if (list_mismatches) *list_mismatches = h[1];
  if ((E->ls.tile_knobs & 32) && E->ls.tile_times.p) {
    unsigned long long t[8];
    ACC_CHECK(hipMemcpy(t, E->ls.tile_times.p, sizeof t, hipMemcpyDeviceToHost));
    const double w = t[5] ? (double)t[5] : 1.0;
    fprintf(stderr, "dbcsr_amd tile kernel, mean per wave [ms]: total %.3f = window waits %.3f + operand waits %.3f + multiplies %.3f + epilogues %.3f + rest %.3f (%llu waves)\n",
            t[0] / w * 1e-5, t[1] / w * 1e-5, t[2] / w * 1e-5, t[3] / w * 1e-5, t[4] / w * 1e-5, ((double)t[0] - t[1] - t[2] - t[3] - t[4]) / w * 1e-5, t[5]);
  }
  if (getenv("DBCSR_AMD_MM_TILE_VERBOSE"))
    fprintf(stderr, "dbcsr_amd tile kernel: %d waves gave up, %lld reads of the team counters, %lld products waited for the window (of %lld)\n", h[0],
            16ll * h[2], 16ll * h[3], (long long)E->facts.nproducts);
  return 0;
}

int dbcsr_amd_mm_band_stats(void* handle, int* waits_gave_up, int* list_mismatches) {
  Engine* E = static_cast<Engine*>(handle);
  if (!E) return -1;
  if (strncmp(E->last_kernel, "mm_numeric_f64_band", 19) != 0 || !E->ls.band_flags.p) return 1;
  int h[4] = {0, 0, 0, 0};
  ACC_CHECK(hipDeviceSynchronize());
  ACC_CHECK(hipMemcpy(h, E->ls.band_flags.p, sizeof h, hipMemcpyDeviceToHost));
  if (waits_gave_up) *waits_gave_up = h[0];
  if (list_mismatches) *list_mismatches = h[1];
  if ((E->ls.band_knobs & 1) && E->ls.band_times.p) {
    unsigned long long t[16];
    ACC_CHECK(hipMemcpy(t, E->ls.band_times.p, sizeof t, hipMemcpyDeviceToHost));
    const double w = t[5] ? (double)t[5] : 1.0;
    fprintf(stderr,
            "dbcsr_amd band kernel, mean per wave [ms]: total %.3f = window waits %.3f + issue and waits for A %.3f + waits for B %.3f + multiplies %.3f + "
            "epilogues %.3f + rest %.3f (%llu waves; %llu of %lld products waited for their B block, %llu fetched it themselves at the last moment; %llu "
            "fetches waited for the window, %llu reads of the team's counters, %d waves switched the throttle off; %lld list entries, shape %d, ring of %d, window %d)\n",
            t[0] / w * 1e-5, t[8] / w * 1e-5, t[1] / w * 1e-5, t[2] / w * 1e-5, t[3] / w * 1e-5, t[4] / w * 1e-5,
            ((double)t[0] - t[1] - t[2] - t[3] - t[4] - t[8]) / w * 1e-5, t[5], t[7], (long long)E->facts.nproducts, t[6], t[9], t[10], h[3], (long long)E->ls.band_nlist,
            E->ls.band_shape, E->ls.band_depth, E->ls.band_window);
  }
  return 0;
}
#endif

#endif
```

### dbcsr_amd/csrc/mm_engine_state.h

```cpp
#ifndef DBCSR_AMD_MM_ENGINE_STATE_H
#define DBCSR_AMD_MM_ENGINE_STATE_H

struct PlanSegs {
  const int32_t* a[12];
  const int32_t* b[12];
  long long n[12];
  int nseg;
};
__global__ void __launch_bounds__(256) plan_compare(PlanSegs S, int* __restrict__ differs) {
  const long long stride = (long long)gridDim.x * blockDim.x;
  bool bad = false;
  for (int g = 0; g < S.nseg; ++g)
    for (long long i = (long long)blockIdx.x * blockDim.x + threadIdx.x; i < S.n[g]; i += stride) bad |= S.a[g][i] != S.b[g][i];
  if (__ballot(bad) && (threadIdx.x & 63) == 0) atomicOr(differs, 1);
}

#ifdef DBCSR_AMD_EXPERIMENTS
struct LabState {
  int group_R = 0;
  bool group_built = false, b_monotone = false;
  int64_t group_panel_bytes = 0;
  DevBuf<int> groups, group_flag, group_cnt;
  DevBuf<GWork> group_work;
  DevBuf<GEntry> group_entries;
  DevBuf<int64_t> group_start;
  int tile_shape = 0;
  int tile_window = 256, tile_rdv = 0, tile_pub = 1, tile_prefetch = 0, tile_knobs = 0;
  bool tile_built = false, band_built = false;
  DevBuf<uint32_t> a_bm, bt_bm, tile_prog;
  DevBuf<unsigned long long> tile_times;
  DevBuf<int> a_pre, tile_rows, tile_cols, tile_cnt, tile_flags;
  DevBuf<int64_t> tile_start;
  DevBuf<TileDesc> tdescs;
  DevBuf<TileEntry> tentries;
  TileGeom tile_geom = {0, 0, 0, 0, 0, 0, 0, 0, 0, 0, 0, 0};
  int band_shape = 1, band_depth = 20, band_bpol = 0, band_knobs = 0, band_window = 384;
  int64_t band_nlist = 0, band_nrem = 0;
  DevBuf<unsigned> band_prog;
  BandGeom band_geom = {0, 0, 0, 0, 0, 0, 0, 0, 0, 0, 0, 0};
  DevBuf<BandDesc> band_descs_buf;
  DevBuf<BandEntry> band_entries;
  DevBuf<BandRem> band_rem;
  DevBuf<int> band_cnt_list, band_cnt_b, band_cnt_rem, band_sub_cnt, band_flags;
  DevBuf<int64_t> band_list_off, band_seq_off, band_rem_start;
  DevBuf<unsigned long long> band_times;
  unsigned hot_xcd_mask = 0xffu;
  DevBuf<unsigned> hot_counters;

  int alg_col_variant = 0;
  int multivec_waves = 0;

  void forget_plan() { tile_built = band_built = group_built = false; }
};
#endif

struct Engine {
  DevBuf<uint32_t> b_bm, c_bm, cin_bm;
  DevBuf<int> b_pre, c_pre, cin_pre, row_nnz, prod_cnt, blk_nze, tmp_i32;
  DevBuf<int64_t> prod_start, c_blk_p_ws, partial, off_a, off_b;
  DevBuf<Entry> entries;
  DevBuf<Desc> descs;
  DevBuf<double> row_sums, norms64;
  DevBuf<float> a_norms, b_norms;
  DevBuf<int> keep;
  DevBuf<int> order, order_cnt;
  DevBuf<int64_t> order_base;
  DevBuf<Work> work;
  DevBuf<unsigned long long> dev_scalars, stat_table;
  int64_t* host_scalars = nullptr;
  DevBuf<int> cls_hist;
  DevBuf<unsigned char> cls_row, cls_col;
  DevBuf<int> cls_vpos, cls_vrow;
  DevBuf<uint32_t> cls_col_bm;
  DevBuf<int64_t> cls_lens;
  int* cls_host_hist = nullptr;
  int64_t* cls_host_lens = nullptr;
  hipEvent_t ev[3] = {nullptr, nullptr, nullptr};
  hipStream_t side_stream[3] = {nullptr, nullptr, nullptr};
  hipEvent_t fork_ev = nullptr, join_ev[3] = {nullptr, nullptr, nullptr};

  SizeFacts facts;
  int W = 0;
  bool have_cin = false, valid = false;
  bool rows_kernels = false;
  bool grid_kernels = false;
  int sym_bitmap = -1, sym_NP = 0, sym_PW = 0, sym_rowp_chunks = 0;
  char last_symbolic[160] = "";
  int64_t cls_len[kNumClasses] = {0}, cls_off[kNumClasses] = {0};
  FilterArgs filter = {nullptr, nullptr, 0.0f};
  double drop_pending = 0.0;
  bool work_built = false;

  const void* norms_data = nullptr;
  int64_t norms_nblks = 0;
  double unwritten_below = 0.0;
  char last_kernel[96] = "";
  bool timed = false;
  int64_t flt_nblks = 0;
  int64_t flt_new_nblks = -1;
  int filter_in_place = 0;
  Window crop_win = {0, 0, 0, 0};
  bool crop_pending = false;
  bool flt_pending = false;
  int twin_mode = -1, twin_nblkrows = 0;
  int64_t twin_nblks = 0;
  KPassMemo kpass_memo;

  DevBuf<double> alg_sums;
  DevBuf<int> alg_i32;
  DevBuf<int64_t> alg_i64;
  DevBuf<uint32_t> alg_bm;
  DevBuf<int> alg_pre, alg_cnt, alg_col_p, alg_list;
  DevBuf<double> alg_vec;
  struct AlgLen {
    const void* rs = nullptr;
    const void* cs = nullptr;
    uint64_t stamp = 0;
    int nbr = 0, nbc = 0;
    int64_t rows = 0;
    int64_t cols = -1;
  };
  static constexpr int kAlgLens = 8;
  AlgLen alg_len[kAlgLens];
  int alg_len_next = 0;
  int add_mode = 0;
  int add_beta_zero = 0;
  int64_t add_nblks_a = 0, add_nblks_b = 0, add_nblks = 0, add_nze = 0;

  DevBuf<int> ew_i32;
  DevBuf<int64_t> ew_i64;
  int had_mode = 0;
  int had_assumed = 0;
  int64_t had_nblks_a = 0, had_nblks_b = 0, had_nblks = 0, had_nze = 0;

  DevBuf<uint32_t> bl_bm;
  DevBuf<unsigned long long> bl_cnt;
  DevBuf<int> bl_i32;
  bool rsv_pending = false;
  const void* rsv_row_p = nullptr;
  int rsv_nblkrows = 0, rsv_nblkcols = 0;
  int64_t rsv_nblks_a = 0, rsv_nblks = 0, rsv_nze = 0;

  DevBuf<int64_t> csr_off;
  DevBuf<int64_t> csr_pos;
  DevBuf<int> csr_slots;
  DevBuf<int> csr_rows;
  DevBuf<int64_t> csr_aux;
  bool csr_pending = false;
  const void *csr_row_p = nullptr, *csr_rs = nullptr, *csr_cs = nullptr;
  int csr_nblkrows = 0, csr_nblkcols = 0, csr_datatype = 0, csr_use_eps = 0;
  int64_t csr_nblks = 0, csr_nnz = 0, csr_nslots = 0;
  double csr_eps = 0.0;
  struct CsrLen {
    const void* row_p = nullptr;
    const void* rs = nullptr;
    const void* cs = nullptr;
    uint64_t stamp = 0;
    int nbr = 0, nbc = 0;
    int64_t nblks = 0, nslots = 0;
    int64_t nze = -1;
  };
  static constexpr int kCsrLens = 8;
// ... 69 lines not shown
```

### dbcsr_amd/csrc/mm_numeric_f64.h

```cpp
#ifndef DBCSR_AMD_MM_NUMERIC_F64_H
#define DBCSR_AMD_MM_NUMERIC_F64_H
#include "mm_epilogue.h"

namespace dbcsr_amd {

template <int MA, int NC>
__device__ __forceinline__ void cblock_f64(const Desc& d, const Entry* __restrict__ entries, const double* __restrict__ a_data,
                                           const double* __restrict__ b_data, double* __restrict__ c_out,
                                           const double* __restrict__ c_in, double alpha, double beta, const LaneMap& L, int row0,
                                           int col0, double* __restrict__ norm_out = nullptr) {
  double acc[MA][NC];
#pragma unroll
  for (int a = 0; a < MA; ++a)
#pragma unroll
    for (int c = 0; c < NC; ++c) acc[a][c] = 0.0;
  const int m = d.m, n = d.n;
  const Entry* e = entries + d.prod_start;
  for (int p = 0; p < d.prod_cnt; ++p) {
    const uint64_t ao = e[p].a_off(), bo = e[p].b_off();
    block_product_f64<MA, NC, false>(acc, a_data + ao, b_data + bo, m, n, e[p].ks(), L, row0, col0);
  }
  double* C = c_out + d.c_off;
  const bool has_in = d.cin_off >= 0;
  const double* Ci = c_in + (has_in ? d.cin_off : 0);
  double ss = 0.0;
#pragma unroll
  for (int a = 0; a < MA; ++a)
#pragma unroll
    for (int c = 0; c < NC; ++c) {
      const int row = row0 + 8 * a + L.rowd, col = col0 + 8 * c + L.coll;
      if (row < m && col < n) {
        double v = alpha * acc[a][c];
        if (has_in) v += beta * Ci[row + (size_t)m * col];
        C[row + (size_t)m * col] = v;
        ss += v * v;
      }
    }
  if (norm_out) {
    ss = wave_sum(ss);
    if ((threadIdx.x & 63) == 0) *norm_out = ss;
  }
}

__global__ void __launch_bounds__(256) mm_numeric_f64(const Desc* __restrict__ descs, int64_t nblk, const Entry* __restrict__ entries,
                                                      const double* __restrict__ a_data, const double* __restrict__ b_data,
                                                      double* __restrict__ c_out, const double* __restrict__ c_in, double alpha,
                                                      double beta, int skip_empty) {
  const int lane = threadIdx.x & 63;
  const int wg = xcd_remap(blockIdx.x, gridDim.x);
  const int64_t cb = __builtin_amdgcn_readfirstlane(wg * 4 + (int)(threadIdx.x >> 6));
  if (cb >= nblk) return;
  const Desc d = descs[cb];
  if (skip_empty && d.prod_cnt == 0) return;
  const LaneMap L(lane);
  const int m = d.m, n = d.n;
  if (m <= 32 && n <= 32) {
    const int MA = (m + 7) >> 3, NC = (n + 7) >> 3;
    switch (MA * 4 + NC) {
#define DBCSR_CASE(A_, C_) \
  case A_ * 4 + C_: cblock_f64<A_, C_>(d, entries, a_data, b_data, c_out, c_in, alpha, beta, L, 0, 0); break;
      DBCSR_CASE(1, 1) DBCSR_CASE(1, 2) DBCSR_CASE(1, 3) DBCSR_CASE(1, 4)
      DBCSR_CASE(2, 1) DBCSR_CASE(2, 2) DBCSR_CASE(2, 3) DBCSR_CASE(2, 4)
      DBCSR_CASE(3, 1) DBCSR_CASE(3, 2) DBCSR_CASE(3, 3) DBCSR_CASE(3, 4)
      DBCSR_CASE(4, 1) DBCSR_CASE(4, 2) DBCSR_CASE(4, 3) DBCSR_CASE(4, 4)
#undef DBCSR_CASE
      default: break;
    }
  } else {
    for (int row0 = 0; row0 < m; row0 += 32)
      for (int col0 = 0; col0 < n; col0 += 32) cblock_f64<4, 4>(d, entries, a_data, b_data, c_out, c_in, alpha, beta, L, row0, col0);
  }
}


template <int MA, int NC>
__device__ __forceinline__ void cblock_f64_lds(const Desc& d, const Entry* __restrict__ entries, const double* __restrict__ a_data,
                                               const double* __restrict__ b_data, double* __restrict__ c_out,
                                               const double* __restrict__ c_in, double alpha, double beta, const LaneMap& L, int lane,
                                               char* lds_a, char* lds_b, int dbg) {
  constexpr int CA = 2 * MA, CB = 2 * NC;
  double acc[MA][NC];
#pragma unroll
  for (int a = 0; a < MA; ++a)
#pragma unroll
    for (int c = 0; c < NC; ++c) acc[a][c] = 0.0;
// ... 162 lines not shown
        if constexpr (VAR == 2 || VAR == 6)
          av[a] = *(lds_vd*)(pa[a] + s * 4 * AP);
        else
          av[a] = pa[a][s * 4 * AP];
      }
#pragma unroll
      for (int c = 0; c < NC; ++c) {
        if constexpr (VAR == 2 || VAR == 6)
          bv[c] = (s == KS - 1 && (K & 3)) ? *(lds_vd*)(pbt[c]) : *(lds_vd*)(pb[c] + 4 * s);
        else
          bv[c] = (s == KS - 1 && (K & 3)) ? pbt[c][0] : pb[c][4 * s];
      }
#pragma unroll
      for (int a = 0; a < MA; ++a)
#pragma unroll
        for (int c = 0; c < NC; ++c) acc[a][c] = __builtin_amdgcn_mfma_f64_4x4x4f64(av[a], bv[c], acc[a][c], 0, 0, 0);
    }
    if constexpr (VAR == 5 || VAR == 6) __builtin_amdgcn_s_setprio(0);
    i0 = i1;
    e0 = e1;
    i1 = i1 + 1;
    e1 = e2;
  }
  for (int p = 0; p < cnt; ++p) {
    const Entry ep = e[p];
    if (ep.ks() != K) block_product_f64<MA, NC, false>(acc, a_data + ep.a_off(), b_data + ep.b_off(), M, N, ep.ks(), L);
  }
  if constexpr (VAR == 3 || VAR == 4) asm volatile("" ::"v"(touch));
  before_epilogue();
  const bool has_in = d.cin_off >= 0;
  if (norm_out && drop_below > 0.0 && !has_in && !(dbg & 8)) {
    const double s2 = acc_norm2<M, N>(acc, alpha, L);
    if (lane == 0) *norm_out = s2;
    if (s2 < drop_below) return;
    norm_out = nullptr;
  }
  if (dbg & 8) {
    double* C = c_out + d.c_off;
    const double* Ci = c_in + (has_in ? d.cin_off : 0);
#pragma unroll
    for (int a = 0; a < MA; ++a)
#pragma unroll
      for (int c = 0; c < NC; ++c) {
        const int row = 8 * a + L.rowd, col = 8 * c + L.coll;
        if (row < M && col < N) {
          double v = alpha * acc[a][c];
          if (has_in) v += beta * Ci[row + (size_t)M * col];
          C[row + (size_t)M * col] = v;
        }
      }
    return;
  }
  stage_c_block<M, N>(reinterpret_cast<double*>(lds_a), acc, alpha, L);
  store_c_block<M, N>(lds_a, c_out + d.c_off, has_in ? c_in + d.cin_off : nullptr, beta, lane, norm_out, !(dbg & 16));
}

template <int M, int N, int K, int VAR>
__global__ void __launch_bounds__(256) mm_numeric_f64_hot(const Desc* __restrict__ descs, int64_t nblk, const Entry* __restrict__ entries,
                                                          const double* __restrict__ a_data, const double* __restrict__ b_data,
                                                          double* __restrict__ c_out, const double* __restrict__ c_in, double alpha,
                                                          double beta, int lds_a_doubles, int lds_wave_doubles, int dbg, const int* __restrict__ order,
                                                          const Work* __restrict__ work, double* __restrict__ norms) {
  extern __shared__ __attribute__((aligned(16))) char smem[];
  const int lane = threadIdx.x & 63;
  const int wid = __builtin_amdgcn_readfirstlane((int)(threadIdx.x >> 6));
  const int wg = xcd_remap(blockIdx.x, gridDim.x);
  const int64_t pos = (int64_t)wg * (int)(blockDim.x >> 6) + wid;
  const Work w = work[pos];
  if (w.prod_cnt < 0) return;
  const double drop_below = norms ? norms[nblk] : 0.0;
  const Desc d = {w.c_off, w.cin_off, w.prod_start, w.prod_cnt, w.m, w.n};
  Entry first;
  first.a_lo = w.a_lo, first.b_lo = w.b_lo, first.w = w.w;
  if ((dbg & 32) && d.prod_cnt == 0) return;
  if ((dbg & 64) && d.m == M && d.n == N) return;
  if constexpr (VAR == 1)
    if ((dbg >> 8) & 0xff & (1 << (blockIdx.x & 7))) return;
  char* lds_a = smem + (size_t)wid * lds_wave_doubles * 8;
  char* lds_b = lds_a + (size_t)lds_a_doubles * 8;
  const LaneMap L(lane);
  if (d.m == M && d.n == N) {
    cblock_f64_exact<M, N, K, VAR>(d, first, entries, a_data, b_data, c_out, c_in, alpha, beta, L, lane, lds_a, lds_b, dbg,
                              norms ? norms + w.cb : nullptr, NoHook(), drop_below);
    return;
  }
  cblock_f64<4, 4>(d, entries, a_data, b_data, c_out, c_in, alpha, beta, L, 0, 0, norms ? norms + w.cb : nullptr);
}

template <int M, int N, int K>
__global__ void __launch_bounds__(64) mm_numeric_f64_hot_persistent(const Entry* __restrict__ entries, const double* __restrict__ a_data,
                                                                    const double* __restrict__ b_data, double* __restrict__ c_out,
                                                                    const double* __restrict__ c_in, double alpha, double beta, int lds_a_doubles,
                                                                    int dbg, const Work* __restrict__ work, long stream_len,
                                                                    unsigned* __restrict__ counters, unsigned xcd_mask, double* __restrict__ norms) {
  extern __shared__ __attribute__((aligned(16))) char smem[];
  const int lane = threadIdx.x & 63;
  const unsigned xcd = blockIdx.x & 7u;
  if (!((xcd_mask >> xcd) & 1u)) return;
  char* lds_a = smem;
  char* lds_b = lds_a + (size_t)lds_a_doubles * 8;
  const LaneMap L(lane);
  const Work* stream = work + (long)xcd * stream_len;
  auto take = [&]() {
    unsigned v = 0;
    if (lane == 0) v = __hip_atomic_fetch_add(&counters[32 * xcd], 1u, __ATOMIC_RELAXED, __HIP_MEMORY_SCOPE_WORKGROUP);
    return v;
  };
  unsigned pos = (unsigned)__builtin_amdgcn_readfirstlane((int)take());
  while ((long)pos < stream_len) {
    const Work w = stream[pos];
    unsigned next_raw = 0;
    if (w.prod_cnt >= 0 && !((dbg & 32) && w.prod_cnt == 0) && w.m == M && w.n == N) {
      const Desc d = {w.c_off, w.cin_off, w.prod_start, w.prod_cnt, w.m, w.n};
      Entry first;
      first.a_lo = w.a_lo, first.b_lo = w.b_lo, first.w = w.w;
      auto hook = [&]() { next_raw = take(); };
      cblock_f64_exact<M, N, K, 0, decltype(hook)>(d, first, entries, a_data, b_data, c_out, c_in, alpha, beta, L, lane, lds_a, lds_b, 0,
                                                   norms ? norms + w.cb : nullptr, hook);
    } else {
      next_raw = take();
      if (w.prod_cnt >= 0 && !((dbg & 32) && w.prod_cnt == 0)) {
        const Desc d = {w.c_off, w.cin_off, w.prod_start, w.prod_cnt, w.m, w.n};
        cblock_f64<4, 4>(d, entries, a_data, b_data, c_out, c_in, alpha, beta, L, 0, 0);
      }
    }
    pos = (unsigned)__builtin_amdgcn_readfirstlane((int)next_raw);
  }
}

template <int MAXT>
__global__ void __launch_bounds__(256) mm_numeric_f64_lds(const Desc* __restrict__ descs, int64_t nblk, const Entry* __restrict__ entries,
                                                          const double* __restrict__ a_data, const double* __restrict__ b_data,
                                                          double* __restrict__ c_out, const double* __restrict__ c_in, double alpha,
                                                          double beta, int lds_a_doubles, int lds_wave_doubles, int dbg, const int* __restrict__ order) {
  extern __shared__ __attribute__((aligned(16))) char smem[];
  const int lane = threadIdx.x & 63;
  const int wid = __builtin_amdgcn_readfirstlane((int)(threadIdx.x >> 6));
  const int wg = xcd_remap(blockIdx.x, gridDim.x);
  const int64_t pos = (int64_t)wg * (int)(blockDim.x >> 6) + wid;
  const int64_t cb = order[pos];
  if (cb < 0 || cb >= nblk) return;
  if ((dbg & 32) && descs[cb].prod_cnt == 0) return;
  char* lds_a = smem + (size_t)wid * lds_wave_doubles * 8;
  char* lds_b = lds_a + (size_t)lds_a_doubles * 8;
  const Desc d = descs[cb];
  const LaneMap L(lane);
  const int MA = (d.m + 7) >> 3, NC = (d.n + 7) >> 3;
  switch (MA * 4 + NC) {
#define DBCSR_CASE(A_, C_)                                                                                           \
  case A_ * 4 + C_:                                                                                                  \
    if constexpr (A_ <= MAXT && C_ <= MAXT)                                                                          \
      cblock_f64_lds<A_, C_>(d, entries, a_data, b_data, c_out, c_in, alpha, beta, L, lane, lds_a, lds_b, dbg);          \
    break;
    DBCSR_CASE(1, 1) DBCSR_CASE(1, 2) DBCSR_CASE(1, 3) DBCSR_CASE(1, 4)
    DBCSR_CASE(2, 1) DBCSR_CASE(2, 2) DBCSR_CASE(2, 3) DBCSR_CASE(2, 4)
    DBCSR_CASE(3, 1) DBCSR_CASE(3, 2) DBCSR_CASE(3, 3) DBCSR_CASE(3, 4)
    DBCSR_CASE(4, 1) DBCSR_CASE(4, 2) DBCSR_CASE(4, 3) DBCSR_CASE(4, 4)
#undef DBCSR_CASE
    default: break;
  }
}


struct PipeCtx {
  const Desc* __restrict__ descs;
  const Entry* __restrict__ entries;
// ... 304 lines not shown
```

### dbcsr_amd/csrc/mm_symbolic.h

```cpp
#ifndef DBCSR_AMD_MM_SYMBOLIC_H
#define DBCSR_AMD_MM_SYMBOLIC_H
#include "mm_epilogue.h"

namespace dbcsr_amd {


__global__ void __launch_bounds__(256) bitmap_from_index(const int* __restrict__ row_p, const int* __restrict__ col_i, int nbr, int W,
                                                         uint32_t* __restrict__ bm) {
  const int lane = threadIdx.x & 63;
  const int row = (blockIdx.x * blockDim.x + threadIdx.x) >> 6;
  if (row >= nbr) return;
  for (int b = row_p[row] + lane; b < row_p[row + 1]; b += 64) {
    const int j = col_i[b];
    atomicOr(&bm[(size_t)row * W + (j >> 5)], 1u << (j & 31));
  }
}

__device__ __forceinline__ uint32_t canonical_bits(int i, int w) {
  const uint32_t even = (i & 1) ? 0xAAAAAAAAu : 0x55555555u;
  const int d = i - 32 * w;
  const uint32_t upper = d <= 0 ? 0xFFFFFFFFu : (d >= 32 ? 0u : ~((1u << d) - 1u));
  return (even & upper) | (~even & ~upper);
}

// ... 167 lines not shown
                                                         const int* __restrict__ b_pre, const uint32_t* __restrict__ cin_bm, int nbr,
                                                         int nbc, int W, int nJ, int retain, int canonical, FilterArgs F,
                                                         uint32_t* __restrict__ c_bm) {
  const int lane = threadIdx.x & 63;
  const int64_t wv = ((int64_t)blockIdx.x * blockDim.x + threadIdx.x) >> 6;
  if (wv >= (int64_t)nbr * nJ) return;
  const int i = (int)(wv / nJ), jb = (int)(wv % nJ);
  const int j = jb * 64 + lane, w = j >> 5, bit = j & 31;
  bool any = false;
  if (!retain && j < nbc && !(canonical && !((canonical_bits(i, w) >> bit) & 1u))) {
    const int a0 = a_row_p[i], a1 = a_row_p[i + 1];
    const float reps = row_filter_eps(F, a1 - a0);
    const uint32_t below = (1u << bit) - 1u;
    for (int ab = a0; ab < a1; ++ab) {
      const int k = a_col_i[ab];
      const uint32_t bw = b_bm[(size_t)k * W + w];
      if ((bw >> bit) & 1u) {
        const int bidx = b_row_p[k] + b_pre[(size_t)k * W + w] + __popc(bw & below);
        if (!(F.a_norms[ab] * F.b_norms[bidx] < reps)) any = true;
      }
    }
  }
  const unsigned long long mask = __ballot(any);
  if (lane == 0) {
    const int w0 = 2 * jb;
    c_bm[(size_t)i * W + w0] = (uint32_t)mask | (cin_bm ? cin_bm[(size_t)i * W + w0] : 0u);
    if (w0 + 1 < W) c_bm[(size_t)i * W + w0 + 1] = (uint32_t)(mask >> 32) | (cin_bm ? cin_bm[(size_t)i * W + w0 + 1] : 0u);
  }
}


__global__ void __launch_bounds__(256) count_products_grid(const int* __restrict__ a_row_p, const int* __restrict__ a_col_i,
                                                           const int* __restrict__ rs, const int* __restrict__ ks,
                                                           const int* __restrict__ cs, const uint32_t* __restrict__ b_bm,
                                                           const uint32_t* __restrict__ c_bm, const int* __restrict__ c_pre,
                                                           const int* __restrict__ c_row_p, int nbr, int nbc, int W, int nJ,
                                                           int* __restrict__ prod_cnt, int* __restrict__ blk_nze,
                                                           unsigned long long* __restrict__ flop_out, const int* __restrict__ b_row_p,
                                                           const int* __restrict__ b_pre, FilterArgs F) {
  const int lane = threadIdx.x & 63;
  const int64_t wv = ((int64_t)blockIdx.x * blockDim.x + threadIdx.x) >> 6;
  unsigned long long flop = 0;
  if (wv < (int64_t)nbr * nJ) {
    const int i = (int)(wv / nJ), jb = (int)(wv % nJ);
    const int j = jb * 64 + lane, w = j >> 5, bit = j & 31;
    const uint32_t cw = w < W ? c_bm[(size_t)i * W + w] : 0u;
    const bool present = (cw >> bit) & 1u;
    if (__ballot(present)) {
      const int a0 = a_row_p[i], a1 = a_row_p[i + 1];
      const float reps = F.a_norms ? row_filter_eps(F, a1 - a0) : 0.0f;
      int cnt = 0;
      long long ksum = 0;
      for (int ab = a0; ab < a1; ++ab) {
        const int k = a_col_i[ab];
        const uint32_t bw = w < W ? b_bm[(size_t)k * W + w] : 0u;
        if ((bw >> bit) & 1u) {
          if (F.a_norms) {
            const int bidx = b_row_p[k] + b_pre[(size_t)k * W + w] + __popc(bw & ((1u << bit) - 1u));
            if (F.a_norms[ab] * F.b_norms[bidx] < reps) continue;
          }
          ++cnt;
          ksum += ks[k];
        }
      }
      if (present) {
        const int cb = c_row_p[i] + c_pre[(size_t)i * W + w] + __popc(cw & ((1u << bit) - 1u));
        const int m = rs[i], n = cs[j];
        prod_cnt[cb] = cnt;
        blk_nze[cb] = m * n;
        flop = 2ull * (unsigned long long)m * n * (unsigned long long)ksum;
      }
    }
  }
  __shared__ unsigned long long red[4];
  flop = wave_sum(flop);
  if ((threadIdx.x & 63) == 0) red[threadIdx.x >> 6] = flop;
  __syncthreads();
  if (threadIdx.x == 0) {
    const unsigned long long t = red[0] + red[1] + red[2] + red[3];
    if (t) atomicAdd(flop_out, t);
  }
}

__global__ void __launch_bounds__(256)
fill_products_grid(const int* __restrict__ a_row_p, const int* __restrict__ a_col_i, const int64_t* __restrict__ a_blk_p,
                   const int* __restrict__ b_row_p, const int64_t* __restrict__ b_blk_p, const int* __restrict__ cin_row_p,
                   const int64_t* __restrict__ cin_blk_p, const int* __restrict__ rs, const int* __restrict__ ks,
                   const int* __restrict__ cs, const uint32_t* __restrict__ b_bm, const int* __restrict__ b_pre,
                   const uint32_t* __restrict__ cin_bm, const int* __restrict__ cin_pre, const uint32_t* __restrict__ c_bm,
                   const int* __restrict__ c_pre, const int* __restrict__ c_row_p, const int64_t* __restrict__ prod_start,
                   const int64_t* __restrict__ c_blk_p_ws, int nbr, int nbc, int W, int nJ, int* __restrict__ c_col_i,
                   int64_t* __restrict__ c_blk_p, Desc* __restrict__ descs, Entry* __restrict__ entries, FilterArgs F) {
  const int lane = threadIdx.x & 63;
  const int64_t wv = ((int64_t)blockIdx.x * blockDim.x + threadIdx.x) >> 6;
  if (wv >= (int64_t)nbr * nJ) return;
  const int i = (int)(wv / nJ), jb = (int)(wv % nJ);
  const int j = jb * 64 + lane, w = j >> 5, bit = j & 31;
  const uint32_t cw = w < W ? c_bm[(size_t)i * W + w] : 0u;
  const bool present = (cw >> bit) & 1u;
  if (!__ballot(present)) return;
  const uint32_t below = (1u << bit) - 1u;
  const int cb = present ? c_row_p[i] + c_pre[(size_t)i * W + w] + __popc(cw & below) : 0;
  const int64_t p0 = present ? prod_start[cb] : 0;
  const int a0 = a_row_p[i], a1 = a_row_p[i + 1];
  const float reps = F.a_norms ? row_filter_eps(F, a1 - a0) : 0.0f;
  int cnt = 0;
  for (int base = a0; base < a1; base += 64) {
    const int top = min(base + 64, a1);
    unsigned long long hits = 0ull;
    for (int ab = base; ab < top; ++ab) {
      const int k = a_col_i[ab];
      const uint32_t bw = w < W ? b_bm[(size_t)k * W + w] : 0u;
      if (present && ((bw >> bit) & 1u)) hits |= 1ull << (ab - base);
    }
    while (hits) {
      const int ab = base + __ffsll((long long)hits) - 1;
      hits &= hits - 1;
      const int k = a_col_i[ab];
      const uint32_t bw = b_bm[(size_t)k * W + w];
      const int bidx = b_row_p[k] + b_pre[(size_t)k * W + w] + __popc(bw & below);
      if (F.a_norms && F.a_norms[ab] * F.b_norms[bidx] < reps) continue;
      entries[p0 + cnt] = Entry::make(a_blk_p[ab], b_blk_p[bidx], ks[k]);
      ++cnt;
    }
  }
  if (present) {
    Desc d;
    d.c_off = c_blk_p_ws[cb];
    d.cin_off = -1;
    if (cin_bm) {
      const uint32_t cinw = cin_bm[(size_t)i * W + w];
      if ((cinw >> bit) & 1u) d.cin_off = cin_blk_p[cin_row_p[i] + cin_pre[(size_t)i * W + w] + __popc(cinw & below)];
    }
    d.prod_start = p0;
    d.prod_cnt = cnt;
    d.m = (int16_t)rs[i];
    d.n = (int16_t)cs[j];
    descs[cb] = d;
    c_col_i[cb] = j;
    c_blk_p[cb] = d.c_off;
  }
}


__global__ void __launch_bounds__(256) c_bitmap_rows_filtered(const int* __restrict__ a_row_p, const int* __restrict__ a_col_i,
                                                              const int* __restrict__ b_row_p, const int* __restrict__ b_col_i, int nbr, int W,
                                                              int canonical, FilterArgs F, uint32_t* __restrict__ c_bm) {
  const int lane = threadIdx.x & 63;
  const int i = (int)(((int64_t)blockIdx.x * blockDim.x + threadIdx.x) >> 6);
  if (i >= nbr) return;
  const float reps = row_filter_eps(F, a_row_p[i + 1] - a_row_p[i]);
  for (int ab = a_row_p[i]; ab < a_row_p[i + 1]; ++ab) {
    const int k = a_col_i[ab];
    for (int bb = b_row_p[k] + lane; bb < b_row_p[k + 1]; bb += 64) {
      if (F.a_norms[ab] * F.b_norms[bb] < reps) continue;
      const int j = b_col_i[bb], w = j >> 5, bit = j & 31;
      if (canonical && !((canonical_bits(i, w) >> bit) & 1u)) continue;
      atomicOr(&c_bm[(size_t)i * W + w], 1u << bit);
    }
  }
}

__global__ void __launch_bounds__(256) count_products_rows(const int* __restrict__ a_row_p, const int* __restrict__ a_col_i,
                                                           const int* __restrict__ rs, const int* __restrict__ ks, const int* __restrict__ cs,
                                                           const int* __restrict__ b_row_p, const int* __restrict__ b_col_i,
                                                           const uint32_t* __restrict__ c_bm, const int* __restrict__ c_pre,
                                                           const int* __restrict__ c_row_p, int nbr, int W, int* __restrict__ prod_cnt,
                                                           unsigned long long* __restrict__ flop_out, FilterArgs F) {
  const int lane = threadIdx.x & 63;
  const int i = (int)(((int64_t)blockIdx.x * blockDim.x + threadIdx.x) >> 6);
  unsigned long long flop = 0;
  if (i < nbr) {
    const unsigned long long m = (unsigned long long)rs[i];
    const float reps = F.a_norms ? row_filter_eps(F, a_row_p[i + 1] - a_row_p[i]) : 0.0f;
    for (int ab = a_row_p[i]; ab < a_row_p[i + 1]; ++ab) {
      const int k = a_col_i[ab];
      const unsigned long long kk = (unsigned long long)ks[k];
      for (int bb = b_row_p[k] + lane; bb < b_row_p[k + 1]; bb += 64) {
        if (F.a_norms && F.a_norms[ab] * F.b_norms[bb] < reps) continue;
        const int j = b_col_i[bb], w = j >> 5, bit = j & 31;
        const uint32_t cw = c_bm[(size_t)i * W + w];
        if (!((cw >> bit) & 1u)) continue;
        const int cb = c_row_p[i] + c_pre[(size_t)i * W + w] + __popc(cw & ((1u << bit) - 1u));
        atomicAdd(&prod_cnt[cb], 1);
        flop += 2ull * m * (unsigned long long)cs[j] * kk;
      }
    }
  }
  __shared__ unsigned long long red[4];
  flop = wave_sum(flop);
  if (lane == 0) red[threadIdx.x >> 6] = flop;
  __syncthreads();
  if (threadIdx.x == 0) {
    const unsigned long long t = red[0] + red[1] + red[2] + red[3];
    if (t) atomicAdd(flop_out, t);
  }
}

__global__ void __launch_bounds__(256) fill_products_rows(const int* __restrict__ a_row_p, const int* __restrict__ a_col_i,
                                                          const int64_t* __restrict__ a_blk_p, const int* __restrict__ ks,
                                                          const int* __restrict__ b_row_p, const int* __restrict__ b_col_i,
                                                          const int64_t* __restrict__ b_blk_p, const uint32_t* __restrict__ c_bm,
                                                          const int* __restrict__ c_pre, const int* __restrict__ c_row_p,
                                                          const int64_t* __restrict__ prod_start, int nbr, int W, int* __restrict__ fill_cnt,
                                                          Entry* __restrict__ entries, FilterArgs F) {
  const int lane = threadIdx.x & 63;
  const int i = (int)(((int64_t)blockIdx.x * blockDim.x + threadIdx.x) >> 6);
  if (i >= nbr) return;
  const float reps = F.a_norms ? row_filter_eps(F, a_row_p[i + 1] - a_row_p[i]) : 0.0f;
  for (int ab = a_row_p[i]; ab < a_row_p[i + 1]; ++ab) {
    const int k = a_col_i[ab];
    const int kk = ks[k];
    const int64_t a_off = a_blk_p[ab];
    for (int bb = b_row_p[k] + lane; bb < b_row_p[k + 1]; bb += 64) {
      if (F.a_norms && F.a_norms[ab] * F.b_norms[bb] < reps) continue;
      const int j = b_col_i[bb], w = j >> 5, bit = j & 31;
      const uint32_t cw = c_bm[(size_t)i * W + w];
      if (!((cw >> bit) & 1u)) continue;
      const int cb = c_row_p[i] + c_pre[(size_t)i * W + w] + __popc(cw & ((1u << bit) - 1u));
      const int slot = atomicAdd(&fill_cnt[cb], 1);
      entries[prod_start[cb] + slot] = Entry::make(a_off, b_blk_p[bb], kk);
    }
  }
}
// ... 107 lines not shown
    d.n = (int16_t)cs[j];
    descs[cb] = d;
    c_col_i[cb] = j;
    c_blk_p[cb] = d.c_off;
    ++cb;
  }
}

template <typename T>
__global__ void __launch_bounds__(256) init_c_blocks(const Desc* __restrict__ descs, int64_t nblk, T* __restrict__ c_out,
                                                     const T* __restrict__ c_in, T beta) {
  const int lane = threadIdx.x & 63;
  const int64_t cb = ((int64_t)blockIdx.x * blockDim.x + threadIdx.x) >> 6;
  if (cb >= nblk) return;
  const Desc d = descs[cb];
  const int ne = (int)d.m * (int)d.n;
  T* C = c_out + d.c_off;
  if (d.cin_off >= 0) {
    const T* Ci = c_in + d.cin_off;
    for (int e = lane; e < ne; e += 64) C[e] = beta * Ci[e];
  } else {
    for (int e = lane; e < ne; e += 64) C[e] = (T)0;
  }
}

__device__ __forceinline__ int panel_rank(const int* __restrict__ c_pre, const int* __restrict__ row_nnz, int i, int W, int w) {
  return w < W ? c_pre[(size_t)i * W + w] : row_nnz[i];
}

__global__ void __launch_bounds__(256) order_count(const int* __restrict__ c_pre, const int* __restrict__ row_nnz, int nbr, int W, int PW,
                                                   int NP, int NG, int RG, int* __restrict__ cnt) {
  const int key = blockIdx.x * blockDim.x + threadIdx.x;
  if (key >= 8 * NP * NG) return;
  const int g = key % NG, p = (key / NG) % NP, x = key / (NG * NP);
  int c = 0;
  for (int t = 0; t < RG; ++t) {
    const int i = 8 * (g * RG + t) + x;
    if (i < nbr) c += panel_rank(c_pre, row_nnz, i, W, (p + 1) * PW) - panel_rank(c_pre, row_nnz, i, W, p * PW);
  }
  cnt[key] = c;
}

__global__ void __launch_bounds__(256) order_fill(const uint32_t* __restrict__ c_bm, const int* __restrict__ c_pre,
                                                  const int* __restrict__ row_nnz, const int* __restrict__ c_row_p,
                                                  const int64_t* __restrict__ base, int nbr, int W, int PW, int NP, int NG, int RG,
                                                  int64_t len, int* __restrict__ order) {
  const int64_t tid = (int64_t)blockIdx.x * blockDim.x + threadIdx.x;
  if (tid >= (int64_t)nbr * W) return;
  const int i = (int)(tid / W), w = (int)(tid % W);
  uint32_t v = c_bm[tid];
  if (!v) return;
  const int x = i & 7, r = i >> 3, g = r / RG, t = r % RG, p = w / PW;
  const int key = (x * NP + p) * NG + g;
  const int64_t dst0 = (int64_t)x * len + (base[key] - base[(size_t)x * NP * NG]);
  const int w0 = p * PW;
  int cb = c_row_p[i] + c_pre[tid];
  while (v) {
    const int bit = __ffs(v) - 1;
    v &= v - 1;
    const uint32_t below = (1u << bit) - 1u;
    int before = 0;
    for (int tt = 0; tt < RG; ++tt) {
      const int ii = 8 * (g * RG + tt) + x;
      if (ii >= nbr) break;
      const uint32_t ww = c_bm[(size_t)ii * W + w];
      before += c_pre[(size_t)ii * W + w] + __popc(ww & below) - panel_rank(c_pre, row_nnz, ii, W, w0);
      if (tt < t) before += (ww >> bit) & 1u;
    }
    order[dst0 + before] = cb;
    ++cb;
  }
}

__global__ void order_len(const int64_t* __restrict__ base, int64_t total, int NP, int NG, int64_t* __restrict__ out) {
  int64_t mx = 0;
  for (int x = 0; x < 8; ++x) {
    const int64_t b0 = base[(size_t)x * NP * NG];
    const int64_t b1 = x < 7 ? base[(size_t)(x + 1) * NP * NG] : total;
    mx = b1 - b0 > mx ? b1 - b0 : mx;
  }
  out[0] = (mx + 3) & ~(int64_t)3;
}


constexpr int kNumClasses = 10;

__global__ void __launch_bounds__(256) class_ids(const int* __restrict__ sizes, int n, int s0, int s1, int s2, unsigned char* __restrict__ cls) {
  const int i = blockIdx.x * blockDim.x + threadIdx.x;
  if (i >= n) return;
  const int s = sizes[i];
  cls[i] = (unsigned char)(s == s0 ? 0 : (s == s1 ? 1 : (s == s2 ? 2 : 3)));
}

__global__ void __launch_bounds__(256) class_col_bitmaps(const unsigned char* __restrict__ ncls, int nbc, int W, uint32_t* __restrict__ bm) {
  const int w = blockIdx.x * blockDim.x + threadIdx.x;
  if (w >= W) return;
  uint32_t m[4] = {0u, 0u, 0u, 0u};
  for (int b = 0; b < 32; ++b) {
    const int j = 32 * w + b;
    if (j < nbc) m[ncls[j]] |= 1u << b;
  }
  for (int q = 0; q < 4; ++q) bm[(size_t)q * W + w] = m[q];
}

__device__ __forceinline__ uint32_t class_mask(int cls, int rc, const uint32_t* __restrict__ ncls_bm, int W, int w) {
  if (cls < 9) return rc == cls / 3 ? ncls_bm[(size_t)(cls % 3) * W + w] : 0u;
  return rc == 3 ? 0xffffffffu : ncls_bm[(size_t)3 * W + w];
}

__global__ void __launch_bounds__(256) class_row_deal(const unsigned char* __restrict__ rowcls, int nbr, int* __restrict__ vpos, int* __restrict__ vrow) {
  __shared__ int cnt[256][4];
  __shared__ int cls_off[4];
  const int t = threadIdx.x, chunk = (nbr + 255) / 256, i0 = t * chunk, i1 = min(nbr, i0 + chunk);
  int c[4] = {0, 0, 0, 0};
  for (int i = i0; i < i1; ++i) ++c[rowcls[i]];
  for (int q = 0; q < 4; ++q) cnt[t][q] = c[q];
  __syncthreads();
  if (t < 4) {
    int run = 0;
    for (int u = 0; u < 256; ++u) {
      const int v = cnt[u][t];
      cnt[u][t] = run;
      run += v;
    }
    cls_off[t] = run;
  }
  __syncthreads();
  if (t == 0) {
    int run = 0;
    for (int q = 0; q < 4; ++q) {
      const int v = cls_off[q];
      cls_off[q] = run;
      run += v;
    }
  }
  __syncthreads();
  int at[4];
  for (int q = 0; q < 4; ++q) at[q] = cls_off[q] + cnt[t][q];
  for (int i = i0; i < i1; ++i) {
    const int j = at[rowcls[i]]++;
    vpos[i] = j;
    vrow[j] = i;
  }
}

__global__ void __launch_bounds__(256) order_count_cls(const uint32_t* __restrict__ c_bm, const unsigned char* __restrict__ rowcls,
                                                       const uint32_t* __restrict__ ncls_bm, const int* __restrict__ vrow, int nbr, int W, int PW, int NP, int R,
                                                       int* __restrict__ cnt) {
  const int key = blockIdx.x * blockDim.x + threadIdx.x;
  if (key >= kNumClasses * 8 * NP * R) return;
  const int g = key % R, p = (key / R) % NP, x = (key / (R * NP)) % 8, cls = key / (R * NP * 8);
  const int j = 8 * g + x;
  int c = 0;
  if (j < nbr) {
    const int i = vrow[j];
    const int rc = rowcls[i];
    const int w1 = min(W, (p + 1) * PW);
    for (int w = p * PW; w < w1; ++w) c += __popc(c_bm[(size_t)i * W + w] & class_mask(cls, rc, ncls_bm, W, w));
  }
  cnt[key] = c;
}

__global__ void order_len_cls(const int64_t* __restrict__ base, int64_t total, int NP, int R, int64_t* __restrict__ lens ) {
  int64_t off = 0;
  for (int cls = 0; cls < kNumClasses; ++cls) {
    int64_t mx = 0;
// ... 54 lines not shown
```

### include/dbcsr_amd_mm.h

```cpp
#ifndef DBCSR_AMD_MM_H
#define DBCSR_AMD_MM_H

#include <stdint.h>

#include "dbcsr_acc_libsmm.h"

#if defined(__cplusplus)
extern "C" {
#endif

typedef struct dbcsr_amd_bcsr {
  int32_t nblkrows, nblkcols;
  const int32_t* row_blk_size;
  const int32_t* col_blk_size;
  int32_t* row_p;
  int32_t* col_i;
  int64_t* blk_p;
  void* data;
  int64_t nblks;
  uint64_t index_stamp;
} dbcsr_amd_bcsr;

typedef struct dbcsr_amd_mm_counts {
  int64_t c_nblks;
// ... 11 lines not shown
int dbcsr_amd_mm_create(void** handle);
int dbcsr_amd_mm_destroy(void* handle);

int dbcsr_amd_mm_symbolic(void* handle, const dbcsr_amd_bcsr* a, const dbcsr_amd_bcsr* b, const dbcsr_amd_bcsr* c_in,
  int retain_sparsity, int32_t* c_out_row_p, dbcsr_amd_mm_counts* counts, void* stream);

int dbcsr_amd_mm_symbolic_filtered(void* handle, libsmm_acc_data_t datatype, double alpha, double filter_eps, const dbcsr_amd_bcsr* a,
  const dbcsr_amd_bcsr* b, const dbcsr_amd_bcsr* c_in, int retain_sparsity, int32_t* c_out_row_p, dbcsr_amd_mm_counts* counts,
  void* stream);

int dbcsr_amd_bcsr_filter_count(void* handle, libsmm_acc_data_t datatype, const dbcsr_amd_bcsr* m, double eps, int32_t* new_row_p,
  int64_t* new_nblks, int64_t* new_nze, void* stream);
int dbcsr_amd_bcsr_filter_apply(void* handle, libsmm_acc_data_t datatype, const dbcsr_amd_bcsr* src, dbcsr_amd_bcsr* dst, void* stream);

int dbcsr_amd_bcsr_filter_apply_index(void* handle, const dbcsr_amd_bcsr* src, dbcsr_amd_bcsr* dst, void* stream);
int dbcsr_amd_mm_set_filter_in_place(void* handle, int on);

int dbcsr_amd_bcsr_crop_count(void* handle, libsmm_acc_data_t datatype, const dbcsr_amd_bcsr* m, int64_t row_lo, int64_t row_hi,
  int64_t col_lo, int64_t col_hi, int32_t* new_row_p, int64_t* new_nblks, int64_t* new_nze, void* stream);
int dbcsr_amd_bcsr_crop_apply(void* handle, libsmm_acc_data_t datatype, const dbcsr_amd_bcsr* src, dbcsr_amd_bcsr* dst, void* stream);
int dbcsr_amd_bcsr_scale_window(void* handle, libsmm_acc_data_t datatype, dbcsr_amd_bcsr* m, double beta, int64_t row_lo,
  int64_t row_hi, int64_t col_lo, int64_t col_hi, void* stream);
int dbcsr_amd_bcsr_scale_window_z(void* handle, dbcsr_amd_bcsr* m, const double beta[2], int64_t row_lo, int64_t row_hi, int64_t col_lo,
  int64_t col_hi, void* stream);

int dbcsr_amd_mm_numeric(void* handle, libsmm_acc_data_t datatype, double alpha, const dbcsr_amd_bcsr* a, const dbcsr_amd_bcsr* b,
  double beta, const dbcsr_amd_bcsr* c_in, dbcsr_amd_bcsr* c_out, void* stream);
int dbcsr_amd_mm_numeric_z(void* handle, const double alpha[2], const dbcsr_amd_bcsr* a, const dbcsr_amd_bcsr* b, const double beta[2],
  const dbcsr_amd_bcsr* c_in, dbcsr_amd_bcsr* c_out, void* stream);

int dbcsr_amd_mm_init_c(void* handle, libsmm_acc_data_t datatype, double beta, const dbcsr_amd_bcsr* c_in, dbcsr_amd_bcsr* c_out,
  void* stream);
int dbcsr_amd_mm_init_c_z(void* handle, const double beta[2], const dbcsr_amd_bcsr* c_in, dbcsr_amd_bcsr* c_out, void* stream);

int dbcsr_amd_bcsr_transpose(void* handle, libsmm_acc_data_t datatype, const dbcsr_amd_bcsr* src, dbcsr_amd_bcsr* dst, void* stream);
int dbcsr_amd_bcsr_transpose_conj(void* handle, libsmm_acc_data_t datatype, const dbcsr_amd_bcsr* src, dbcsr_amd_bcsr* dst, void* stream);

int dbcsr_amd_bcsr_checksum(void* handle, libsmm_acc_data_t datatype, const dbcsr_amd_bcsr* m, double* out2, void* stream);

int dbcsr_amd_bcsr_fill_random(void* handle, libsmm_acc_data_t datatype, const dbcsr_amd_bcsr* m, int counter, void* stream);

int dbcsr_amd_bcsr_fill_random_dist(void* handle, libsmm_acc_data_t datatype, const dbcsr_amd_bcsr* m, int counter,
  const int32_t* row_gid, const int32_t* col_gid, int32_t nblkrows_global, void* stream);

int dbcsr_amd_multiply(void* handle, char transa, char transb, libsmm_acc_data_t datatype, double alpha, const dbcsr_amd_bcsr* matrix_a,
  const dbcsr_amd_bcsr* matrix_b, double beta, const dbcsr_amd_bcsr* matrix_c, const int64_t* limits, int retain_sparsity,
  double filter_eps, dbcsr_amd_bcsr* c_out, int64_t* flop, void* stream);
int dbcsr_amd_multiply_z(void* handle, char transa, char transb, const double alpha[2], const dbcsr_amd_bcsr* matrix_a, const dbcsr_amd_bcsr* matrix_b,
  const double beta[2], const dbcsr_amd_bcsr* matrix_c, const int64_t* limits, int retain_sparsity, double filter_eps,
  dbcsr_amd_bcsr* c_out, int64_t* flop, void* stream);
int dbcsr_amd_bcsr_release(dbcsr_amd_bcsr* m);

int dbcsr_amd_mm_timing(void* handle, float* ms_fill, float* ms_numeric);

int dbcsr_amd_bcsr_desymmetrize_count(void* handle, const dbcsr_amd_bcsr* src, int32_t* dst_row_p, int64_t* nblks, int64_t* nze, void* stream);
int dbcsr_amd_bcsr_desymmetrize_apply(void* handle, libsmm_acc_data_t datatype, const dbcsr_amd_bcsr* src, int kind, dbcsr_amd_bcsr* dst, void* stream);

int dbcsr_amd_bcsr_desymmetrized(void* handle, libsmm_acc_data_t datatype, const dbcsr_amd_bcsr* src, int kind, dbcsr_amd_bcsr* dst, void* stream);
int dbcsr_amd_bcsr_twin_count(void* handle, const dbcsr_amd_bcsr* src, int mode, int32_t* dst_row_p, int64_t* nblks, int64_t* nze, void* stream);
int dbcsr_amd_bcsr_twin_apply(void* handle, libsmm_acc_data_t datatype, const dbcsr_amd_bcsr* src, int mode, int kind, dbcsr_amd_bcsr* dst,
  void* stream);
int dbcsr_amd_mm_set_canonical_product(void* handle, int on);
int dbcsr_amd_multiply_symmetric_c(void* handle, char transa, char transb, libsmm_acc_data_t datatype, double alpha,
  const dbcsr_amd_bcsr* matrix_a, const dbcsr_amd_bcsr* matrix_b, double beta, const dbcsr_amd_bcsr* matrix_c, int kind,
  int retain_sparsity, double filter_eps, dbcsr_amd_bcsr* c_out, int64_t* flop, void* stream);
int dbcsr_amd_multiply_symmetric_c_klimits(void* handle, char transa, char transb, libsmm_acc_data_t datatype, double alpha,
  const dbcsr_amd_bcsr* matrix_a, const dbcsr_amd_bcsr* matrix_b, double beta, const dbcsr_amd_bcsr* matrix_c, int kind,
  int64_t first_k, int64_t last_k, int retain_sparsity, double filter_eps, dbcsr_amd_bcsr* c_out, int64_t* flop, void* stream);
int dbcsr_amd_multiply_symmetric_c_z(void* handle, char transa, char transb, const double alpha[2], const dbcsr_amd_bcsr* matrix_a,
  const dbcsr_amd_bcsr* matrix_b, const double beta[2], const dbcsr_amd_bcsr* matrix_c, int kind, int64_t first_k, int64_t last_k,
  int retain_sparsity, double filter_eps, dbcsr_amd_bcsr* c_out, int64_t* flop, void* stream);

int dbcsr_amd_mm_stats(void* handle, dbcsr_amd_mnk_stat* out, int max_entries, int* n_entries, void* stream);

const char* dbcsr_amd_mm_kernel_name(libsmm_acc_data_t datatype);
const char* dbcsr_amd_mm_last_kernel(void* handle);
const char* dbcsr_amd_mm_last_symbolic(void* handle);
const char* dbcsr_amd_smm_last_kernel(void);

int dbcsr_amd_mm_trust_plan(void* handle, int on);

int dbcsr_amd_mm_expect_filter(void* handle, double eps);
int dbcsr_amd_mm_plan_stats(void* handle, int64_t* reused, int64_t* built);

int dbcsr_amd_bcsr_add_count(void* handle, const dbcsr_amd_bcsr* a, const dbcsr_amd_bcsr* b, int beta_is_zero, int32_t* dst_row_p, int64_t* nblks,
  int64_t* nze, int* same_pattern, void* stream);
int dbcsr_amd_bcsr_add_apply(void* handle, libsmm_acc_data_t datatype, const double alpha[2], const dbcsr_amd_bcsr* a, const double beta[2],
  const dbcsr_amd_bcsr* b, dbcsr_amd_bcsr* dst, void* stream);
int dbcsr_amd_bcsr_diag_count(void* handle, const dbcsr_amd_bcsr* m, int32_t* dst_row_p, int32_t* dst_col_i, int64_t* dst_blk_p, int64_t* nblks,
  int64_t* nze, void* stream);
int dbcsr_amd_bcsr_diag_fill(void* handle, libsmm_acc_data_t datatype, const double alpha[2], dbcsr_amd_bcsr* dst, void* stream);
int dbcsr_amd_bcsr_diag_shift(void* handle, libsmm_acc_data_t datatype, dbcsr_amd_bcsr* m, const double alpha[2], void* stream);
int dbcsr_amd_bcsr_trace(void* handle, libsmm_acc_data_t datatype, const dbcsr_amd_bcsr* m, double out[2], void* stream);
int dbcsr_amd_bcsr_dot(void* handle, libsmm_acc_data_t datatype, const dbcsr_amd_bcsr* a, const dbcsr_amd_bcsr* b, int symmetric, double out[1],
  void* stream);
int dbcsr_amd_bcsr_norm2(void* handle, libsmm_acc_data_t datatype, const dbcsr_amd_bcsr* m, int symmetric, double out[1], void* stream);

int dbcsr_amd_bcsr_maxabs(void* handle, libsmm_acc_data_t datatype, const dbcsr_amd_bcsr* m, double out[1], void* stream);
int dbcsr_amd_bcsr_row_sums(void* handle, libsmm_acc_data_t datatype, const dbcsr_amd_bcsr* m, int what, double* out, int64_t n_out, void* stream);
int dbcsr_amd_bcsr_col_sums(void* handle, libsmm_acc_data_t datatype, const dbcsr_amd_bcsr* m, int what, int skip_diagonal_blocks, double* out,
  int64_t n_out, void* stream);
int dbcsr_amd_bcsr_gershgorin(void* handle, libsmm_acc_data_t datatype, const dbcsr_amd_bcsr* m, int symmetric, double out[1], void* stream);
int dbcsr_amd_bcsr_get_diag(void* handle, libsmm_acc_data_t datatype, const dbcsr_amd_bcsr* m, void* diag, int64_t n, void* stream);
int dbcsr_amd_bcsr_set_diag(void* handle, libsmm_acc_data_t datatype, dbcsr_amd_bcsr* m, const void* diag, int64_t n, void* stream);
int dbcsr_amd_bcsr_scale_by_vector(void* handle, libsmm_acc_data_t datatype, dbcsr_amd_bcsr* m, const void* vec, int64_t n, int side, void* stream);
int dbcsr_amd_bcsr_matvec(void* handle, libsmm_acc_data_t datatype, char trans, const double alpha[2], const dbcsr_amd_bcsr* a,
  int kind , const void* x, int64_t n_x, const double beta[2], void* y, int64_t n_y, void* stream);
int dbcsr_amd_bcsr_multivec(void* handle, libsmm_acc_data_t datatype, char trans, const double alpha[2], const dbcsr_amd_bcsr* a,
  int kind , int nrhs, const void* x, int64_t n_x, int64_t ldx, const double beta[2], void* y, int64_t n_y, int64_t ldy,
  void* stream);
int dbcsr_amd_bcsr_rank_update(void* handle, libsmm_acc_data_t datatype, char trans, const double alpha[2], int nrhs, const void* x, int64_t n_x,
  int64_t ldx, const void* y, int64_t n_y, int64_t ldy, const double beta[2], dbcsr_amd_bcsr* a, void* stream);

int dbcsr_amd_bcsr_block_diag_count(void* handle, const dbcsr_amd_bcsr* m, int32_t* dst_row_p, int32_t* dst_col_i, int64_t* dst_blk_p,
  int64_t* nblks, int64_t* nze, int32_t* max_dim, void* stream);
int dbcsr_amd_bcsr_block_diag_apply(void* handle, libsmm_acc_data_t datatype, const dbcsr_amd_bcsr* src, dbcsr_amd_bcsr* dst, void* stream);
int dbcsr_amd_bcsr_block_diag_invert(void* handle, libsmm_acc_data_t datatype, dbcsr_amd_bcsr* m, int max_dim, int64_t info[3], void* stream);

int dbcsr_amd_bcsr_block_diag_multiply(void* handle, libsmm_acc_data_t datatype, char side , char trans, const double alpha[2],
  const dbcsr_amd_bcsr* diag, dbcsr_amd_bcsr* m, int max_dim, void* stream);

int dbcsr_amd_bcsr_to_dense(void* handle, libsmm_acc_data_t datatype, const dbcsr_amd_bcsr* m, int kind , void* dense,
  int64_t n_rows, int64_t n_cols, int64_t ld, int col_major, void* stream);
int dbcsr_amd_bcsr_from_dense_apply(void* handle, libsmm_acc_data_t datatype, const void* dense, int64_t n_rows, int64_t n_cols, int64_t ld, int col_major,
  dbcsr_amd_bcsr* m, void* stream);
int dbcsr_amd_bcsr_from_dense_count(void* handle, libsmm_acc_data_t datatype, const void* dense, int64_t n_rows, int64_t n_cols, int64_t ld, int col_major,
  const int32_t* row_blk_size, const int32_t* col_blk_size, int nblkrows, int nblkcols, double eps, int32_t* dst_row_p, int32_t* dst_col_i,
  int64_t* dst_blk_p, int64_t* nblks, int64_t* nze, void* stream);

int dbcsr_amd_bcsr_submatrix_gather(void* handle, libsmm_acc_data_t datatype, const dbcsr_amd_bcsr* m, int kind, int nsub, const int32_t* set_ptr,
  const int32_t* set_idx, const int32_t* set_off, const int32_t* sub_dim, int nslot, const int32_t* slot_sub, int max_members, void* dense, int64_t n,
  int64_t ld, int64_t batch_stride, double pad_diag, void* stream);
int dbcsr_amd_bcsr_submatrix_scatter(void* handle, libsmm_acc_data_t datatype, const void* dense, int64_t n, int64_t ld, int64_t batch_stride, int nsub,
  const int32_t* set_ptr, const int32_t* set_idx, const int32_t* set_off, const int32_t* owner, const int32_t* sub_slot, dbcsr_amd_bcsr* m,
  void* stream);

int dbcsr_amd_bcsr_hadamard_count(void* handle, const dbcsr_amd_bcsr* a, const dbcsr_amd_bcsr* b, int b_assumed, int32_t* dst_row_p, int64_t* nblks,
  int64_t* nze, int* same_pattern, void* stream);
int dbcsr_amd_bcsr_hadamard_apply(void* handle, libsmm_acc_data_t datatype, const dbcsr_amd_bcsr* a, const dbcsr_amd_bcsr* b,
  const double b_value[2] , dbcsr_amd_bcsr* dst, void* stream);
int dbcsr_amd_bcsr_copy_onto(void* handle, libsmm_acc_data_t datatype, const dbcsr_amd_bcsr* src, dbcsr_amd_bcsr* dst, void* stream);
enum {
  dbcsr_func_inverse = 0, dbcsr_func_tanh = 1, dbcsr_func_dtanh = 2, dbcsr_func_ddtanh = 3, dbcsr_func_artanh = 4, dbcsr_func_sin = 7,
  dbcsr_func_dsin = 8, dbcsr_func_ddsin = 9, dbcsr_func_asin = 10, dbcsr_func_cos = 11, dbcsr_func_dcos = 12, dbcsr_func_ddcos = 13
};
int dbcsr_amd_bcsr_function_of_elements(void* handle, libsmm_acc_data_t datatype, dbcsr_amd_bcsr* m, int func, double a0, double a1, void* stream);

int dbcsr_amd_bcsr_reserve_count(void* handle, const dbcsr_amd_bcsr* m, int64_t n, const int32_t* rows, const int32_t* cols, int upper_only,
  int32_t* dst_row_p, int64_t* nblks, int64_t* nze, int64_t* n_new, int64_t* n_invalid, void* stream);
int dbcsr_amd_bcsr_reserve_apply(void* handle, libsmm_acc_data_t datatype, const dbcsr_amd_bcsr* m, dbcsr_amd_bcsr* dst, void* stream);
int dbcsr_amd_bcsr_put_blocks(void* handle, libsmm_acc_data_t datatype, dbcsr_amd_bcsr* m, int64_t n, const int32_t* rows, const int32_t* cols,
  const int64_t* src_off, const void* src, const double alpha[2], int summation, void* stream);
int dbcsr_amd_bcsr_get_blocks(void* handle, libsmm_acc_data_t datatype, const dbcsr_amd_bcsr* m, int64_t n, const int32_t* rows, const int32_t* cols,
  const int64_t* dst_off, void* dst, int32_t* found, void* stream);

int dbcsr_amd_bcsr_to_csr_count(void* handle, libsmm_acc_data_t datatype, const dbcsr_amd_bcsr* m, int use_eps, double eps, int64_t* crow, int64_t* nnz,
  void* stream);
int dbcsr_amd_bcsr_to_csr_apply(void* handle, libsmm_acc_data_t datatype, const dbcsr_amd_bcsr* m, int32_t* col, void* values, void* stream);
int dbcsr_amd_bcsr_from_csr(void* handle, libsmm_acc_data_t datatype, int64_t n_rows, int64_t n_cols, int64_t nnz, const int64_t* crow, const int32_t* col,
  const void* values, dbcsr_amd_bcsr* m, void* stream);
int dbcsr_amd_bcsr_csr_name_blocks(void* handle, int64_t n_rows, int64_t nnz, const int64_t* crow, const int32_t* col, const int32_t* row_blk_size,
  const int32_t* col_blk_size, int nblkrows, int nblkcols, int32_t* rows, int32_t* cols, void* stream);

int dbcsr_amd_fabric_probe(double* stream_tb_per_s, double* gather_tb_per_s);

#if defined(__cplusplus)
// ... 4 lines not shown
```

Measured before the change: 38080 GFLOP/s.

## Pipeline product-list construction with hot f64 numeric kernel panel by panel

For large fp64 hot-cube multiplies, the C column space is split into panels. Panel 0's product lists and work records are built on the main stream; later panels are built on a side stream with a capped grid, and each panel's numeric kernel waits on an event for its own lists. The goal is to overlap the symbolic fill and work-build phases with numeric compute instead of running them back to back. In exchange it adds events, a small device-to-host copy of panel boundaries, more kernel launches, and shares the GPU between the side-stream fill and the numeric kernels.

```diff
diff --git a/dbcsr_amd/csrc/mm_aux.h b/dbcsr_amd/csrc/mm_aux.h
--- a/dbcsr_amd/csrc/mm_aux.h
+++ b/dbcsr_amd/csrc/mm_aux.h
@@ -1,6 +1,7 @@
 #ifndef DBCSR_AMD_MM_AUX_H
 #define DBCSR_AMD_MM_AUX_H
 #include "mm_epilogue.h"
+#include "mm_panels.h"
 
 namespace dbcsr_amd {
 
@@ -489,11 +490,7 @@
 
 
 constexpr int kStatSlots = 8192;
-__global__ void __launch_bounds__(256) build_work(const int* __restrict__ order, int64_t npos, const Desc* __restrict__ descs, int64_t nblk,
-                                                  const Entry* __restrict__ entries, Work* __restrict__ work) {
-  const int64_t pos = (int64_t)blockIdx.x * blockDim.x + threadIdx.x;
-  if (pos >= npos) return;
-  const int cb = order[pos];
+__device__ __forceinline__ Work work_record(int cb, const Desc* __restrict__ descs, int64_t nblk, const Entry* __restrict__ entries) {
   Work w;
   w.c_off = 0, w.cin_off = -1, w.prod_start = 0, w.prod_cnt = -1, w.m = 0, w.n = 0, w.a_lo = 0, w.b_lo = 0, w.w = 0, w.cb = cb;
   if (cb >= 0 && cb < nblk) {
@@ -504,7 +501,25 @@
       w.a_lo = e.a_lo, w.b_lo = e.b_lo, w.w = e.w;
     }
   }
-  work[pos] = w;
+  return w;
+}
+
+__global__ void __launch_bounds__(256) build_work(const int* __restrict__ order, int64_t npos, const Desc* __restrict__ descs, int64_t nblk,
+                                                  const Entry* __restrict__ entries, Work* __restrict__ work) {
+  const int64_t pos = (int64_t)blockIdx.x * blockDim.x + threadIdx.x;
+  if (pos >= npos) return;
+  work[pos] = work_record(order[pos], descs, nblk, entries);
+}
+
+__global__ void __launch_bounds__(256) build_work_panel(const int* __restrict__ order, PanelSeg seg, int64_t len, int64_t span, int pad_tail,
+                                                        const Desc* __restrict__ descs, int64_t nblk, const Entry* __restrict__ entries,
+                                                        Work* __restrict__ work) {
+  const int x = blockIdx.y;
+  const int64_t l = (int64_t)blockIdx.x * blockDim.x + threadIdx.x;
+  if (l >= span) return;
+  if (!panel_valid(seg, x, l) && !(pad_tail && seg.start[x] + l < len)) return;
+  const int64_t pos = panel_position(seg, len, x, l);
+  work[pos] = work_record(order[pos], descs, nblk, entries);
 }
 
 __global__ void __launch_bounds__(256) mnk_histogram(const Desc* __restrict__ descs, int64_t nblk, const Entry* __restrict__ entries,
diff --git a/dbcsr_amd/csrc/mm_choose.h b/dbcsr_amd/csrc/mm_choose.h
--- a/dbcsr_amd/csrc/mm_choose.h
+++ b/dbcsr_amd/csrc/mm_choose.h
@@ -78,6 +78,9 @@
   int use_mid = 1;
   int use_big = 1;
   int use_work = 1;
+  int pipeline = 1;
+  int64_t pipeline_min_blocks = 2000000;
+  int pipeline_side_blocks = 256;
   int use_classes = 1;
   int wg_waves = 0;
   int f32_direct = 1;
diff --git a/dbcsr_amd/csrc/mm_engine.hip b/dbcsr_amd/csrc/mm_engine.hip
--- a/dbcsr_amd/csrc/mm_engine.hip
+++ b/dbcsr_amd/csrc/mm_engine.hip
@@ -11,6 +11,7 @@
 #include "common.h"
 #include "smm_core.h"
 #include "mm_types.h"
+#include "mm_panels.h"
 #include "mm_complex.h"
 #include "mm_jit.h"
 
@@ -52,6 +53,17 @@
 #endif
 
 
+static void launch_fill_grid(Engine* E, const dbcsr_amd_bcsr* a, const dbcsr_amd_bcsr* b, const dbcsr_amd_bcsr* c_in, dbcsr_amd_bcsr* c_out, hipStream_t st,
+                             int w0, int w1, int max_blocks = 0) {
+  const int nbr = E->facts.nbr, nJ = (w1 - 1) / 2 - w0 / 2 + 1;
+  dim3 grid = grid_for((int64_t)nbr * nJ * 64);
+  if (max_blocks > 0) grid.x = std::min<unsigned>(grid.x, (unsigned)max_blocks);
+  hipLaunchKernelGGL(fill_products_grid, grid, dim3(256), 0, st, a->row_p, a->col_i, a->blk_p, b->row_p, b->blk_p,
+                     c_in->row_p, c_in->blk_p, a->row_blk_size, a->col_blk_size, b->col_blk_size, E->b_bm.p, E->b_pre.p,
+                     E->have_cin ? E->cin_bm.p : nullptr, E->have_cin ? E->cin_pre.p : nullptr, E->c_bm.p, E->c_pre.p, c_out->row_p, E->prod_start.p,
+                     E->c_blk_p_ws.p, nbr, b->nblkcols, E->W, nJ, c_out->col_i, c_out->blk_p, E->descs.p, E->entries.p, E->filter, w0, w1);
+}
+
 static int build_product_lists(Engine* E, bool reuse, const dbcsr_amd_bcsr* a, const dbcsr_amd_bcsr* b, const dbcsr_amd_bcsr* c_in, dbcsr_amd_bcsr* c_out,
                                hipStream_t st) {
   const int nbr = E->facts.nbr, W = E->W, nbc = b->nblkcols, nJ = (nbc + 63) / 64;
@@ -70,10 +82,7 @@
                        c_out->col_blk_size, cin_bm, cin_pre, E->c_bm.p, E->c_pre.p, c_out->row_p, E->c_blk_p_ws.p, E->prod_start.p,
                        E->prod_cnt.p, nbr, W, nJ, c_out->col_i, c_out->blk_p, E->descs.p);
   } else if (E->grid_kernels) {
-    hipLaunchKernelGGL(fill_products_grid, grid_for((int64_t)nbr * nJ * 64), dim3(256), 0, st, a->row_p, a->col_i, a->blk_p, b->row_p,
-                       b->blk_p, c_in->row_p, c_in->blk_p, a->row_blk_size, a->col_blk_size, b->col_blk_size, E->b_bm.p, E->b_pre.p,
-                       cin_bm, cin_pre, E->c_bm.p, E->c_pre.p, c_out->row_p, E->prod_start.p, E->c_blk_p_ws.p, nbr, nbc, W, nJ, c_out->col_i,
-                       c_out->blk_p, E->descs.p, E->entries.p, E->filter);
+    launch_fill_grid(E, a, b, c_in, c_out, st, 0, W);
   } else {
     hipLaunchKernelGGL(fill_products, grid_for((int64_t)nbr * W), dim3(256), 0, st, a->row_p, a->col_i, a->blk_p, b->row_p, b->blk_p,
                        c_in->row_p, c_in->blk_p, a->row_blk_size, a->col_blk_size, b->col_blk_size, E->b_bm.p, E->b_pre.p,
@@ -211,6 +220,70 @@
   return launch_z64(p, c, z64_tiles(F.max_m), z64_tiles(F.max_n), 8 * F.order_len) ? 0 : -1;
 }
 
+struct PanelPlan {
+  int NP = 0, PW = 0;
+  PanelSeg seg[kMaxPipelinePanels];
+  int64_t Lp[kMaxPipelinePanels];
+};
+
+static void launch_panel_lists(Engine* E, const PanelPlan& P, int p, const dbcsr_amd_bcsr* a, const dbcsr_amd_bcsr* b, const dbcsr_amd_bcsr* c_in,
+                               dbcsr_amd_bcsr* c_out, hipStream_t st) {
+  const int64_t len = E->facts.order_len;
+  const bool last = p == P.NP - 1;
+  if (P.Lp[p] > 0) launch_fill_grid(E, a, b, c_in, c_out, st, p * P.PW, std::min((p + 1) * P.PW, E->W), p > 0 ? E->sw.pipeline_side_blocks : 0);
+  int64_t span = P.Lp[p];
+  if (last)
+    for (int x = 0; x < kPanelXcds; ++x) span = std::max<int64_t>(span, len - P.seg[p].start[x]);
+  if (span > 0)
+    hipLaunchKernelGGL(build_work_panel, dim3((unsigned)((span + 255) / 256), kPanelXcds), dim3(256), 0, st, E->order.p, P.seg[p], len, span, last ? 1 : 0,
+                       E->descs.p, E->facts.c_nblks, E->entries.p, E->work.p);
+}
+
+static int pipelined_hot_f64_body(Engine* E, const NumericChoice& c, const NumericArgs<double>& p, const PanelPlan& P, const dbcsr_amd_bcsr* a,
+                                  const dbcsr_amd_bcsr* b, const dbcsr_amd_bcsr* c_in, dbcsr_amd_bcsr* c_out, int* launches) {
+  const SizeFacts& F = E->facts;
+  hipStream_t side = E->side_stream[0];
+  for (int q = 1; q < P.NP; ++q) {
+    launch_panel_lists(E, P, q, a, b, c_in, c_out, side);
+    ACC_CHECK(hipEventRecord(E->ready_ev[q], side));
+  }
+  ACC_CHECK(hipEventRecord(E->ev[1], p.st));
+  for (int q = 0; q < P.NP; ++q) {
+    if (q > 0) ACC_CHECK(hipStreamWaitEvent(p.st, E->ready_ev[q], 0));
+    if (P.Lp[q] == 0) continue;
+    if (!launch_hot_f64_panel(p, c, F.hot_m, F.hot_n, F.hot_k, c.flags, P.seg[q], P.Lp[q], F.order_len)) return -1;
+    ++*launches;
+  }
+  return check(hipGetLastError(), "dbcsr_amd_mm_numeric (panel launches)", __FILE__, __LINE__);
+}
+
+static int pipelined_hot_f64(Engine* E, const NumericChoice& c, const NumericArgs<double>& p, const dbcsr_amd_bcsr* a, const dbcsr_amd_bcsr* b,
+                             const dbcsr_amd_bcsr* c_in, dbcsr_amd_bcsr* c_out) {
+  snprintf(E->last_kernel, sizeof E->last_kernel, "%s", c.name);
+  if (p.norms && c.leaves_norms) E->norms_data = p.c_out, E->norms_nblks = p.nblk;
+  PanelPlan P;
+  P.NP = E->sym_NP, P.PW = E->sym_PW;
+  for (int q = 0; q < P.NP; ++q) P.Lp[q] = panel_segment(E->panel_host, P.NP, q, c.ww, &P.seg[q]);
+  if (!E->fork_ev) ACC_CHECK(hipEventCreateWithFlags(&E->fork_ev, hipEventDisableTiming));
+  if (!E->side_stream[0]) {
+    ACC_CHECK(hipStreamCreateWithFlags(&E->side_stream[0], hipStreamNonBlocking));
+    ACC_CHECK(hipEventCreateWithFlags(&E->join_ev[0], hipEventDisableTiming));
+  }
+  for (int q = 1; q < P.NP; ++q)
+    if (!E->ready_ev[q]) ACC_CHECK(hipEventCreateWithFlags(&E->ready_ev[q], hipEventDisableTiming));
+  launch_panel_lists(E, P, 0, a, b, c_in, c_out, p.st);
+  ACC_CHECK(hipEventRecord(E->fork_ev, p.st));
+  ACC_CHECK(hipStreamWaitEvent(E->side_stream[0], E->fork_ev, 0));
+  int launches = 0;
+  const int rc = pipelined_hot_f64_body(E, c, p, P, a, b, c_in, c_out, &launches);
+  ACC_CHECK(hipEventRecord(E->join_ev[0], E->side_stream[0]));
+  ACC_CHECK(hipStreamWaitEvent(p.st, E->join_ev[0], 0));
+  if (rc) return rc;
+  const size_t at = strlen(E->last_kernel);
+  snprintf(E->last_kernel + at, sizeof E->last_kernel - at, " in %d panel launches", launches);
+  return 0;
+}
+
 static int numeric_phase(void* handle, libsmm_acc_data_t datatype, const double alpha[2], const dbcsr_amd_bcsr* a, const dbcsr_amd_bcsr* b,
                          const double beta[2], const dbcsr_amd_bcsr* c_in, dbcsr_amd_bcsr* c_out, void* stream);
 
@@ -233,6 +306,8 @@
       hipHostMalloc(reinterpret_cast<void**>(&E->cls_host_lens), (2 * kNumClasses + 1) * sizeof(int64_t), hipHostMallocDefault) != hipSuccess)
     return -1;
   if (hipHostMalloc(reinterpret_cast<void**>(&E->plan_host_flag), sizeof(int), hipHostMallocDefault) != hipSuccess) return -1;
+  if (hipHostMalloc(reinterpret_cast<void**>(&E->panel_host), panel_gathered_count(kMaxPipelinePanels) * sizeof(int64_t), hipHostMallocDefault) != hipSuccess)
+    return -1;
   engine_read_env(E);
   for (int i = 0; i < 3; ++i) {
     e = hipEventCreate(&E->ev[i]);
@@ -261,6 +336,9 @@
   if (E->plan_host_flag) (void)hipHostFree(E->plan_host_flag);
   if (E->cls_host_hist) (void)hipHostFree(E->cls_host_hist);
   if (E->cls_host_lens) (void)hipHostFree(E->cls_host_lens);
+  if (E->panel_host) (void)hipHostFree(E->panel_host);
+  for (int i = 0; i < kMaxPipelinePanels; ++i)
+    if (E->ready_ev[i]) (void)hipEventDestroy(E->ready_ev[i]);
   for (int i = 0; i < 3; ++i)
     if (E->ev[i]) (void)hipEventDestroy(E->ev[i]);
   for (int i = 0; i < 3; ++i) {
@@ -314,6 +392,7 @@
   }
   plan_invalidate(E);
   E->valid = false;
+  E->panels_gathered = false;
   E->facts.nbr = nbr;
   E->facts.nbc = nbc;
   E->W = W;
@@ -461,6 +540,12 @@
   hipLaunchKernelGGL(order_count, grid_for(nkeys), dim3(256), 0, st, E->c_pre.p, E->row_nnz.p, nbr, W, PW, NP, NG, RG, E->order_cnt.p);
   if (exclusive_scan<int64_t>(E, E->order_cnt.p, nkeys, E->order_base.p, nullptr, false, st)) return -1;
   hipLaunchKernelGGL(order_len, dim3(1), dim3(1), 0, st, E->order_base.p, c_nblks, NP, NG, dsc + 7);
+  if (E->sw.pipeline && NP >= 2 && NP <= kMaxPipelinePanels) {
+    if (E->panel_base.ensure((size_t)panel_gathered_count(kMaxPipelinePanels))) return -1;
+    hipLaunchKernelGGL(panel_gather, grid_for(panel_gathered_count(NP)), dim3(256), 0, st, E->order_base.p, c_nblks, NP, NG, E->panel_base.p);
+    ACC_CHECK(hipMemcpyAsync(E->panel_host, E->panel_base.p, sizeof(int64_t) * (size_t)panel_gathered_count(NP), hipMemcpyDeviceToHost, st));
+    E->panels_gathered = true;
+  }
   }
   if (E->prod_cnt.ensure((size_t)c_nblks + 1) || E->blk_nze.ensure((size_t)c_nblks + 1) || E->prod_start.ensure((size_t)c_nblks + 1) ||
       E->c_blk_p_ws.ensure((size_t)c_nblks + 1))
@@ -572,21 +657,26 @@
 #endif
   }
   if (E->entries.ensure((size_t)F.nproducts + 1) || E->descs.ensure((size_t)nblk + 1)) return -1;
-  ACC_CHECK(hipEventRecord(E->ev[0], st));
-  if (int rc = build_product_lists(E, reuse, a, b, c_in, c_out, st)) return rc;
   F.nbc = b->nblkcols;
   F.fp64 = datatype == dbcsr_type_real_8;
   F.cplx = datatype == dbcsr_type_complex_8;
   F.filter_active = E->filter.a_norms != nullptr;
   F.skip_empty = (c_out->data == c_in->data && F.retain && beta == 1.0 && beta_z[1] == 0.0) ? 1 : 0;
   const NumericChoice ch = choose_numeric(F, E->sw, E->lab);
+  const bool pipelined = !reuse && E->sw.pipeline && E->panels_gathered && E->grid_kernels && F.fp64 && !F.cplx && ch.family == Family::f64_hot &&
+                         ch.work && ch.variant == 0 && nblk >= E->sw.pipeline_min_blocks;
+  ACC_CHECK(hipEventRecord(E->ev[0], st));
+  if (!pipelined)
+    if (int rc = build_product_lists(E, reuse, a, b, c_in, c_out, st)) return rc;
   const Work* work = nullptr;
   if (ch.work) {
     const int64_t npos = 8 * F.order_len;
     if (!(reuse && E->work_built)) {
       if (E->work.ensure((size_t)npos + 1)) return -1;
-      hipLaunchKernelGGL(build_work, grid_for(npos), dim3(256), 0, st, E->order.p, npos, E->descs.p, nblk, E->entries.p, E->work.p);
-      E->work_built = true;
+      if (!pipelined) {
+        hipLaunchKernelGGL(build_work, grid_for(npos), dim3(256), 0, st, E->order.p, npos, E->descs.p, nblk, E->entries.p, E->work.p);
+        E->work_built = true;
+      }
     }
     work = E->work.p;
   }
@@ -603,8 +693,14 @@
     hipLaunchKernelGGL(store_scalar_f64, dim3(1), dim3(1), 0, st, norms + nblk, drop);
     E->unwritten_below = drop;
   }
-  ACC_CHECK(hipEventRecord(E->ev[1], st));
-  if ((F.cplx ? launch_z64_family(E, ch, numeric_args<z64>(E, st, a, b, c_in, c_out, z64(alpha, alpha_z[1]), z64(beta, beta_z[1]), work, norms, reuse))
+  if (!pipelined) ACC_CHECK(hipEventRecord(E->ev[1], st));
+  if (pipelined) {
+    if (pipelined_hot_f64(E, ch, numeric_args<double>(E, st, a, b, c_in, c_out, alpha, beta, work, norms, reuse), a, b, c_in, c_out) != 0) {
+      fprintf(stderr, "dbcsr_amd_mm_numeric: launching %s panel by panel failed\n", E->last_kernel);
+      return -1;
+    }
+    E->work_built = true;
+  } else if ((F.cplx ? launch_z64_family(E, ch, numeric_args<z64>(E, st, a, b, c_in, c_out, z64(alpha, alpha_z[1]), z64(beta, beta_z[1]), work, norms, reuse))
        : F.fp64 ? launch_f64(E, ch, numeric_args<double>(E, st, a, b, c_in, c_out, alpha, beta, work, norms, reuse), E->lab)
                 : launch_f32(E, ch, numeric_args<float>(E, st, a, b, c_in, c_out, (float)alpha, (float)beta, work, norms, reuse))) != 0) {
     fprintf(stderr, "dbcsr_amd_mm_numeric: launching %s failed\n", E->last_kernel);
diff --git a/dbcsr_amd/csrc/mm_engine_env.h b/dbcsr_amd/csrc/mm_engine_env.h
--- a/dbcsr_amd/csrc/mm_engine_env.h
+++ b/dbcsr_amd/csrc/mm_engine_env.h
@@ -12,6 +12,9 @@
   if (const char* k = getenv("DBCSR_AMD_MM_PIPE_G")) E->sw.pipe_g = std::max(1, atoi(k));
   if (const char* k = getenv("DBCSR_AMD_MM_CLASSES")) E->sw.use_classes = atoi(k);
   if (const char* k = getenv("DBCSR_AMD_MM_WORK")) E->sw.use_work = atoi(k);
+  if (const char* k = getenv("DBCSR_AMD_MM_PIPELINE")) E->sw.pipeline = atoi(k);
+  if (const char* k = getenv("DBCSR_AMD_MM_PIPELINE_SIDE_BLOCKS")) E->sw.pipeline_side_blocks = std::max(0, atoi(k));
+  if (const char* k = getenv("DBCSR_AMD_MM_PIPELINE_MIN_BLOCKS")) E->sw.pipeline_min_blocks = std::max(0ll, atoll(k));
   if (const char* k = getenv("DBCSR_AMD_MM_WG_WAVES")) {
     const int w = atoi(k);
     if (w == 1 || w == 2 || w == 4) E->sw.wg_waves = w;
diff --git a/dbcsr_amd/csrc/mm_engine_launch.h b/dbcsr_amd/csrc/mm_engine_launch.h
--- a/dbcsr_amd/csrc/mm_engine_launch.h
+++ b/dbcsr_amd/csrc/mm_engine_launch.h
@@ -59,6 +59,22 @@
   case S_:                                                                                                                                          \
     hipLaunchKernelGGL((mm_numeric_f64_hot<S_, S_, S_, 0>), grid, block, c.lds_bytes, p.st, p.descs, p.nblk, p.entries, p.a, p.b, p.c_out, p.c_in,  \
                        p.alpha, p.beta, c.lds_a, c.lds_wave, flags, p.order, p.work, p.norms);                                                     \
+    return true;
+    DBCSR_AMD_HOT_SIZES(DBCSR_HOT_CASE)
+#undef DBCSR_HOT_CASE
+    default: return false;
+  }
+}
+
+static bool launch_hot_f64_panel(const NumericArgs<double>& p, const NumericChoice& c, int m, int n, int k, int flags, const PanelSeg& seg, int64_t Lp,
+                                 int64_t len) {
+  if (!hot_f64_has(m, n, k)) return false;
+  const dim3 grid((unsigned)panel_grid(Lp, c.ww)), block(64 * c.ww);
+  switch (m) {
+#define DBCSR_HOT_CASE(S_)                                                                                                                          \
+  case S_:                                                                                                                                          \
+    hipLaunchKernelGGL((mm_numeric_f64_hot_panel<S_, S_, S_>), grid, block, c.lds_bytes, p.st, p.descs, p.nblk, p.entries, p.a, p.b, p.c_out,       \
+                       p.c_in, p.alpha, p.beta, c.lds_a, c.lds_wave, flags, p.work, p.norms, seg, len);                                            \
     return true;
     DBCSR_AMD_HOT_SIZES(DBCSR_HOT_CASE)
 #undef DBCSR_HOT_CASE
diff --git a/dbcsr_amd/csrc/mm_engine_ops.h b/dbcsr_amd/csrc/mm_engine_ops.h
--- a/dbcsr_amd/csrc/mm_engine_ops.h
+++ b/dbcsr_amd/csrc/mm_engine_ops.h
@@ -519,6 +519,36 @@
   return 0;
 }
 
+int dbcsr_amd_mm_lists_differ(void* handle, void* other, int* differ, void* stream) {
+  Engine* E = static_cast<Engine*>(handle);
+  Engine* O = static_cast<Engine*>(other);
+  if (!E || !O || !differ || !E->valid || !O->valid) return -1;
+  const SizeFacts &F = E->facts, &G = O->facts;
+  if (F.c_nblks != G.c_nblks || F.nproducts != G.nproducts || F.order_len != G.order_len || E->work_built != O->work_built) {
+    *differ = 1;
+    return 0;
+  }
+  hipStream_t st = stream_of(stream);
+  DevBuf<int> flag;
+  if (flag.ensure(1)) return -1;
+  ACC_CHECK(hipMemsetAsync(flag.p, 0, sizeof(int), st));
+  PlanSegs S = {};
+  S.a[0] = reinterpret_cast<const int32_t*>(E->entries.p), S.b[0] = reinterpret_cast<const int32_t*>(O->entries.p);
+  S.n[0] = (long long)F.nproducts * (long long)(sizeof(Entry) / 4);
+  S.a[1] = reinterpret_cast<const int32_t*>(E->descs.p), S.b[1] = reinterpret_cast<const int32_t*>(O->descs.p);
+  S.n[1] = (long long)F.c_nblks * (long long)(sizeof(Desc) / 4);
+  S.nseg = 2;
+  if (E->work_built) {
+    S.a[2] = reinterpret_cast<const int32_t*>(E->work.p), S.b[2] = reinterpret_cast<const int32_t*>(O->work.p);
+    S.n[2] = 8 * (long long)F.order_len * (long long)(sizeof(Work) / 4);
+    S.nseg = 3;
+  }
+  hipLaunchKernelGGL(plan_compare, dim3(1024), dim3(256), 0, st, S, flag.p);
+  ACC_CHECK(hipMemcpyAsync(differ, flag.p, sizeof(int), hipMemcpyDeviceToHost, st));
+  ACC_CHECK(hipStreamSynchronize(st));
+  return 0;
+}
+
 int dbcsr_amd_mm_plan_stats(void* handle, int64_t* reused, int64_t* built) {
   Engine* E = static_cast<Engine*>(handle);
   if (!E) return -1;
diff --git a/dbcsr_amd/csrc/mm_engine_state.h b/dbcsr_amd/csrc/mm_engine_state.h
--- a/dbcsr_amd/csrc/mm_engine_state.h
+++ b/dbcsr_amd/csrc/mm_engine_state.h
@@ -78,6 +78,10 @@
   hipEvent_t ev[3] = {nullptr, nullptr, nullptr};
   hipStream_t side_stream[3] = {nullptr, nullptr, nullptr};
   hipEvent_t fork_ev = nullptr, join_ev[3] = {nullptr, nullptr, nullptr};
+  DevBuf<int64_t> panel_base;
+  int64_t* panel_host = nullptr;
+  bool panels_gathered = false;
+  hipEvent_t ready_ev[kMaxPipelinePanels] = {nullptr};
 
   SizeFacts facts;
   int W = 0;
diff --git a/dbcsr_amd/csrc/mm_numeric_f64.h b/dbcsr_amd/csrc/mm_numeric_f64.h
--- a/dbcsr_amd/csrc/mm_numeric_f64.h
+++ b/dbcsr_amd/csrc/mm_numeric_f64.h
@@ -1,6 +1,7 @@
 #ifndef DBCSR_AMD_MM_NUMERIC_F64_H
 #define DBCSR_AMD_MM_NUMERIC_F64_H
 #include "mm_epilogue.h"
+#include "mm_panels.h"
 
 namespace dbcsr_amd {
 
@@ -329,6 +330,36 @@
   if (d.m == M && d.n == N) {
     cblock_f64_exact<M, N, K, VAR>(d, first, entries, a_data, b_data, c_out, c_in, alpha, beta, L, lane, lds_a, lds_b, dbg,
                               norms ? norms + w.cb : nullptr, NoHook(), drop_below);
+    return;
+  }
+  cblock_f64<4, 4>(d, entries, a_data, b_data, c_out, c_in, alpha, beta, L, 0, 0, norms ? norms + w.cb : nullptr);
+}
+
+template <int M, int N, int K>
+__global__ void __launch_bounds__(256) mm_numeric_f64_hot_panel(const Desc* __restrict__ descs, int64_t nblk, const Entry* __restrict__ entries,
+                                                                const double* __restrict__ a_data, const double* __restrict__ b_data,
+                                                                double* __restrict__ c_out, const double* __restrict__ c_in, double alpha,
+                                                                double beta, int lds_a_doubles, int lds_wave_doubles, int dbg,
+                                                                const Work* __restrict__ work, double* __restrict__ norms, PanelSeg seg, int64_t len) {
+  extern __shared__ __attribute__((aligned(16))) char smem[];
+  const int lane = threadIdx.x & 63;
+  const int wid = __builtin_amdgcn_readfirstlane((int)(threadIdx.x >> 6));
+  const int x = blockIdx.x & 7;
+  const int64_t l = (int64_t)(blockIdx.x >> 3) * (int)(blockDim.x >> 6) + wid;
+  if (!panel_valid(seg, x, l)) return;
+  const Work w = work[panel_position(seg, len, x, l)];
+  if (w.prod_cnt < 0) return;
+  const double drop_below = norms ? norms[nblk] : 0.0;
+  const Desc d = {w.c_off, w.cin_off, w.prod_start, w.prod_cnt, w.m, w.n};
+  Entry first;
+  first.a_lo = w.a_lo, first.b_lo = w.b_lo, first.w = w.w;
+  if ((dbg & 32) && d.prod_cnt == 0) return;
+  char* lds_a = smem + (size_t)wid * lds_wave_doubles * 8;
+  char* lds_b = lds_a + (size_t)lds_a_doubles * 8;
+  const LaneMap L(lane);
+  if (d.m == M && d.n == N) {
+    cblock_f64_exact<M, N, K, 0>(d, first, entries, a_data, b_data, c_out, c_in, alpha, beta, L, lane, lds_a, lds_b, dbg, norms ? norms + w.cb : nullptr,
+                                 NoHook(), drop_below);
     return;
   }
   cblock_f64<4, 4>(d, entries, a_data, b_data, c_out, c_in, alpha, beta, L, 0, 0, norms ? norms + w.cb : nullptr);
diff --git a/dbcsr_amd/csrc/mm_panels.h b/dbcsr_amd/csrc/mm_panels.h
--- /dev/null
+++ b/dbcsr_amd/csrc/mm_panels.h
@@ -0,0 +1,43 @@
+#ifndef DBCSR_AMD_MM_PANELS_H
+#define DBCSR_AMD_MM_PANELS_H
+
+#include <cstdint>
+
+#if defined(__HIPCC__)
+#define DBCSR_AMD_PANELS_HD __host__ __device__
+#else
+#define DBCSR_AMD_PANELS_HD
+#endif
+
+namespace dbcsr_amd {
+
+constexpr int kPanelXcds = 8;
+constexpr int kMaxPipelinePanels = 32;
+
+struct PanelSeg {
+  int32_t start[kPanelXcds];
+  int32_t n[kPanelXcds];
+};
+
+static inline int panel_gathered_count(int NP) { return kPanelXcds * NP + 1; }
+
+static inline int64_t panel_segment(const int64_t* gathered, int NP, int p, int ww, PanelSeg* seg) {
+  int64_t longest = 0;
+  for (int x = 0; x < kPanelXcds; ++x) {
+    const int64_t first = gathered[(int64_t)x * NP], lo = gathered[(int64_t)x * NP + p], hi = gathered[(int64_t)x * NP + p + 1];
+    seg->start[x] = (int32_t)(lo - first);
+    seg->n[x] = (int32_t)(hi - lo);
+    longest = hi - lo > longest ? hi - lo : longest;
+  }
+  return (longest + ww - 1) / ww * ww;
+}
+
+static inline int64_t panel_grid(int64_t Lp, int ww) { return kPanelXcds * Lp / ww; }
+
+DBCSR_AMD_PANELS_HD static inline bool panel_valid(const PanelSeg& seg, int x, int64_t l) { return l < (int64_t)seg.n[x]; }
+DBCSR_AMD_PANELS_HD static inline int64_t panel_position(const PanelSeg& seg, int64_t len, int x, int64_t l) {
+  return (int64_t)x * len + seg.start[x] + l;
+}
+
+}
+#endif
diff --git a/dbcsr_amd/csrc/mm_symbolic.h b/dbcsr_amd/csrc/mm_symbolic.h
--- a/dbcsr_amd/csrc/mm_symbolic.h
+++ b/dbcsr_amd/csrc/mm_symbolic.h
@@ -273,21 +273,19 @@
   }
 }
 
-__global__ void __launch_bounds__(256)
-fill_products_grid(const int* __restrict__ a_row_p, const int* __restrict__ a_col_i, const int64_t* __restrict__ a_blk_p,
+__device__ __forceinline__ void
+fill_products_wave(const int* __restrict__ a_row_p, const int* __restrict__ a_col_i, const int64_t* __restrict__ a_blk_p,
                    const int* __restrict__ b_row_p, const int64_t* __restrict__ b_blk_p, const int* __restrict__ cin_row_p,
                    const int64_t* __restrict__ cin_blk_p, const int* __restrict__ rs, const int* __restrict__ ks,
                    const int* __restrict__ cs, const uint32_t* __restrict__ b_bm, const int* __restrict__ b_pre,
                    const uint32_t* __restrict__ cin_bm, const int* __restrict__ cin_pre, const uint32_t* __restrict__ c_bm,
                    const int* __restrict__ c_pre, const int* __restrict__ c_row_p, const int64_t* __restrict__ prod_start,
                    const int64_t* __restrict__ c_blk_p_ws, int nbr, int nbc, int W, int nJ, int* __restrict__ c_col_i,
-                   int64_t* __restrict__ c_blk_p, Desc* __restrict__ descs, Entry* __restrict__ entries, FilterArgs F) {
-  const int lane = threadIdx.x & 63;
-  const int64_t wv = ((int64_t)blockIdx.x * blockDim.x + threadIdx.x) >> 6;
-  if (wv >= (int64_t)nbr * nJ) return;
-  const int i = (int)(wv / nJ), jb = (int)(wv % nJ);
+                   int64_t* __restrict__ c_blk_p, Desc* __restrict__ descs, Entry* __restrict__ entries, FilterArgs F, int w0, int w1, int64_t wv) {
+  const int lane = threadIdx.x & 63;
+  const int i = (int)(wv / nJ), jb = w0 / 2 + (int)(wv % nJ);
   const int j = jb * 64 + lane, w = j >> 5, bit = j & 31;
-  const uint32_t cw = w < W ? c_bm[(size_t)i * W + w] : 0u;
+  const uint32_t cw = w >= w0 && w < w1 ? c_bm[(size_t)i * W + w] : 0u;
   const bool present = (cw >> bit) & 1u;
   if (!__ballot(present)) return;
   const uint32_t below = (1u << bit) - 1u;
@@ -331,6 +329,21 @@
     c_col_i[cb] = j;
     c_blk_p[cb] = d.c_off;
   }
+}
+
+__global__ void __launch_bounds__(256)
+fill_products_grid(const int* __restrict__ a_row_p, const int* __restrict__ a_col_i, const int64_t* __restrict__ a_blk_p,
+                   const int* __restrict__ b_row_p, const int64_t* __restrict__ b_blk_p, const int* __restrict__ cin_row_p,
+                   const int64_t* __restrict__ cin_blk_p, const int* __restrict__ rs, const int* __restrict__ ks,
+                   const int* __restrict__ cs, const uint32_t* __restrict__ b_bm, const int* __restrict__ b_pre,
+                   const uint32_t* __restrict__ cin_bm, const int* __restrict__ cin_pre, const uint32_t* __restrict__ c_bm,
+                   const int* __restrict__ c_pre, const int* __restrict__ c_row_p, const int64_t* __restrict__ prod_start,
+                   const int64_t* __restrict__ c_blk_p_ws, int nbr, int nbc, int W, int nJ, int* __restrict__ c_col_i,
+                   int64_t* __restrict__ c_blk_p, Desc* __restrict__ descs, Entry* __restrict__ entries, FilterArgs F, int w0, int w1) {
+  const int64_t nwaves = (int64_t)nbr * nJ, stride = ((int64_t)gridDim.x * blockDim.x) >> 6;
+  for (int64_t wv = ((int64_t)blockIdx.x * blockDim.x + threadIdx.x) >> 6; wv < nwaves; wv += stride)
+    fill_products_wave(a_row_p, a_col_i, a_blk_p, b_row_p, b_blk_p, cin_row_p, cin_blk_p, rs, ks, cs, b_bm, b_pre, cin_bm, cin_pre, c_bm, c_pre, c_row_p,
+                       prod_start, c_blk_p_ws, nbr, nbc, W, nJ, c_col_i, c_blk_p, descs, entries, F, w0, w1, wv);
 }
 
 
@@ -604,6 +617,12 @@
   out[0] = (mx + 3) & ~(int64_t)3;
 }
 
+__global__ void __launch_bounds__(256) panel_gather(const int64_t* __restrict__ base, int64_t total, int NP, int NG, int64_t* __restrict__ out) {
+  const int t = blockIdx.x * blockDim.x + threadIdx.x;
+  if (t > 8 * NP) return;
+  out[t] = t < 8 * NP ? base[(size_t)t * NG] : total;
+}
+
 
 constexpr int kNumClasses = 10;
 
diff --git a/include/dbcsr_amd_mm.h b/include/dbcsr_amd_mm.h
--- a/include/dbcsr_amd_mm.h
+++ b/include/dbcsr_amd_mm.h
@@ -117,6 +117,7 @@
 
 int dbcsr_amd_mm_expect_filter(void* handle, double eps);
 int dbcsr_amd_mm_plan_stats(void* handle, int64_t* reused, int64_t* built);
+int dbcsr_amd_mm_lists_differ(void* handle, void* other, int* differ, void* stream);
 
 int dbcsr_amd_bcsr_add_count(void* handle, const dbcsr_amd_bcsr* a, const dbcsr_amd_bcsr* b, int beta_is_zero, int32_t* dst_row_p, int64_t* nblks,
   int64_t* nze, int* same_pattern, void* stream);
```

Result: slower. 37510 GFLOP/s (-1.5%).
